# 101001000/ElevenRender

Hardware: AMD Instinct MI355X
Metric: Msamples/sec (rays traced x bounces) at 1920x1080, 1M-tri scene (higher is better)
Workload: dtype f32; 1 GPU; C2: 1000000-triangle random soup + 2048x1024 sky HDRI, 1920x1080, max_bounces 8, 1 step = 1 spp pass (config total 256 spp), seed 12345; schedule=stream

## Files before the change

elevenrender_amd/abi.py:

```python
import ctypes as C
import os

import numpy as np

_HERE = os.path.dirname(os.path.abspath(__file__))
LIB_PATH = os.environ.get("ELEVEN_HIP_LIB") or os.path.join(_HERE, "libeleven_hip.so")

ER_OK = 0
ER_ERR_INVALID_ARG, ER_ERR_NO_DEVICE, ER_ERR_HIP, ER_ERR_STATE, ER_ERR_OOM = -1, -2, -3, -4, -5
PASS_BEAUTY, PASS_DENOISE, PASS_NORMAL, PASS_TANGENT, PASS_BITANGENT, PASS_COUNT = 0, 1, 2, 3, 4, 5
PASS_NAMES = {"beauty": 0, "denoise": 1, "normal": 2, "tangent": 3, "bitangent": 4}
FLAG_POINT_LIGHTS, FLAG_COUNTERS, FLAG_MEGAKERNEL, FLAG_PROFILE, FLAG_FUSED, FLAG_WAVEFRONT, FLAG_GPU_BUILD, FLAG_MIS, FLAG_STREAM = 1, 2, 4, 8, 16, 32, 64, 128, 256
FLAG_HOST_BUILD = 512
FLAG_MESH_LIGHTS = 1024


class ErVec3(C.Structure):
    _fields_ = [("x", C.c_float), ("y", C.c_float), ("z", C.c_float)]


class ErCamera(C.Structure):
    _fields_ = [("focal_length", C.c_float), ("sensor_width", C.c_float), ("sensor_height", C.c_float),
                ("aperture", C.c_float), ("focus_distance", C.c_float), ("rotation", ErVec3),
                ("bokeh", C.c_int32), ("position", ErVec3)]


class ErMaterial(C.Structure):
    _fields_ = [("albedo_tex", C.c_int32), ("emission_tex", C.c_int32), ("roughness_tex", C.c_int32),
                ("metallic_tex", C.c_int32), ("normal_tex", C.c_int32), ("opacity_tex", C.c_int32),
                ("transmission_tex", C.c_int32), ("albedo_shader_id", C.c_int32),
                ("albedo", ErVec3), ("emission", ErVec3),
                ("opacity", C.c_float), ("roughness", C.c_float), ("metallic", C.c_float),
                ("clearcoat_gloss", C.c_float), ("clearcoat", C.c_float), ("anisotropic", C.c_float),
                ("eta", C.c_float), ("transmission", C.c_float), ("specular", C.c_float),
                ("specular_tint", C.c_float), ("sheen_tint", C.c_float), ("subsurface", C.c_float),
                ("sheen", C.c_float), ("ax", C.c_float), ("ay", C.c_float)]


class ErTexture(C.Structure):
    _fields_ = [("width", C.c_int32), ("height", C.c_int32), ("channels", C.c_int32), ("filter", C.c_int32),
                ("data", C.POINTER(C.c_float))]


class ErHdri(C.Structure):
    _fields_ = [("texture", ErTexture), ("cdf", C.POINTER(C.c_float)), ("radiance_sum", C.c_float)]


class ErPointLight(C.Structure):
    _fields_ = [("position", ErVec3), ("radiance", ErVec3)]


class ErSceneDesc(C.Structure):
    _fields_ = [("tri_count", C.c_uint32),
                ("vertices", C.POINTER(C.c_float)), ("normals", C.POINTER(C.c_float)),
                ("tangents", C.POINTER(C.c_float)), ("uvs", C.POINTER(C.c_float)),
                ("tangent_sign", C.POINTER(C.c_float)), ("material_id", C.POINTER(C.c_int32)),
                ("material_count", C.c_uint32), ("materials", C.POINTER(ErMaterial)),
                ("texture_count", C.c_uint32), ("textures", C.POINTER(ErTexture)),
                ("hdri", ErHdri), ("camera", ErCamera),
                ("point_light_count", C.c_uint32), ("point_lights", C.POINTER(ErPointLight)),
                ("x_res", C.c_uint32), ("y_res", C.c_uint32)]


class ErRenderParams(C.Structure):
    _fields_ = [("sample_target", C.c_uint32), ("block_size", C.c_uint32), ("max_bounces", C.c_uint32),
                ("device", C.c_int32), ("rank", C.c_uint32), ("world", C.c_uint32), ("flags", C.c_uint32)]


class ErDeviceInfo(C.Structure):
    _fields_ = [("name", C.c_char * 256), ("platform", C.c_char * 64), ("memory_bytes", C.c_uint64),
                ("compute_units", C.c_uint32), ("compatible", C.c_int32), ("arch", C.c_char * 64)]


class ErCounters(C.Structure):
    _fields_ = [(n, C.c_uint64) for n in ("paths", "bounce_samples", "rays", "node_visits", "tri_tests",
                                          "shaded_hits", "texel_fetches", "hdri_samples", "trace_wave_steps", "trace_busy_lanes",
                                          "trace_node_lanes", "trace_tri_lanes")]


class ErProfile(C.Structure):
    _fields_ = [("trace_ms", C.c_float), ("shade_ms", C.c_float), ("trace_launches", C.c_uint32), ("shade_launches", C.c_uint32), ("schedule", C.c_uint32),
                ("concurrency", C.c_uint32), ("empty_launches", C.c_uint32), ("empty_ms", C.c_float), ("rays_logged", C.c_uint64)]


class ErAccelInfo(C.Structure):
    _fields_ = [("node_count", C.c_uint32), ("node_bytes", C.c_uint32), ("leaf_count", C.c_uint32),
                ("max_depth", C.c_uint32), ("tri_record_bytes", C.c_uint32), ("build_ms", C.c_float),
                ("upload_ms", C.c_float), ("lift_bound", C.c_float), ("builder", C.c_uint32)]


class ErAdaptiveParams(C.Structure):
    _fields_ = [("threshold", C.c_float), ("min_samples", C.c_uint32), ("interval", C.c_uint32)]


class ErAdaptiveInfo(C.Structure):
    _fields_ = [("enabled", C.c_uint32), ("owned_tiles", C.c_uint32), ("active_tiles", C.c_uint32), ("tests_done", C.c_uint32),
                ("samples_rendered", C.c_uint32), ("next_test", C.c_uint32), ("pixel_samples", C.c_uint64), ("max_active_error", C.c_float)]


class ErLightInfo(C.Structure):
    _fields_ = [("emitters", C.c_uint32), ("total_weight", C.c_float)]


class ErStreamInfo(C.Structure):
    _fields_ = [("waves", C.c_uint32), ("tracers", C.c_uint32), ("large_regions", C.c_uint32), ("deal_pending", C.c_uint32), ("launches", C.c_uint32),
                ("pixels_per_cu", C.c_uint32), ("lanes_busy", C.c_double), ("launch_ms", C.c_double), ("cost_spread", C.c_double),
                ("spec_started", C.c_uint64), ("spec_right", C.c_uint64), ("spec_wrong", C.c_uint64),
                ("form", C.c_uint32), ("reserved", C.c_uint32)]


class ErStreamForm(C.Structure):
    _fields_ = [("waves", C.c_uint32), ("tracers", C.c_uint32), ("adapt", C.c_uint32), ("keep", C.c_uint32), ("spec", C.c_uint32), ("reserved", C.c_uint32)]


class ErAccelDump(C.Structure):
    _fields_ = [("tri_count", C.c_uint32), ("node_count", C.c_uint32), ("node8_count", C.c_uint32), ("node8_pieces", C.c_uint32),
                ("attr_pieces", C.c_uint32), ("max_depth", C.c_uint32), ("max_depth8", C.c_uint32), ("builder", C.c_uint32),
                ("lo", C.c_float * 3), ("hi", C.c_float * 3), ("lift_bound", C.c_float), ("max_lift", C.c_float)]


NODE_DTYPE = np.dtype([("lo0", "<f4", 3), ("hi0", "<f4", 3), ("lo1", "<f4", 3), ("hi1", "<f4", 3), ("c0", "<i4"), ("c1", "<i4"), ("pad", "<i4", 2)])
NODE8_DTYPE = np.dtype([("p", "<f4", 3), ("e", "u1", 3), ("imask", "u1"), ("child_base", "<u4"), ("tri_base", "<u4"), ("tri_present", "<u4"),
                        ("reserved", "<u4"), ("qlo", "u1", (3, 8)), ("qhi", "u1", (3, 8))])
ISECT_DTYPE = np.dtype([("v0", "<f4", 3), ("tri_id", "<i4"), ("v1", "<f4", 3), ("lift", "<f4"), ("v2", "<f4", 3), ("sign", "<f4")])
assert NODE_DTYPE.itemsize == 64 and NODE8_DTYPE.itemsize == 80 and ISECT_DTYPE.itemsize == 48


def attr_dtype(pieces):
    dt = np.dtype([("n", "<f4", (3, 3)), ("t", "<f4", (3, 3)), ("uv", "<f4", (3, 2)), ("material", "<i4"), ("pad", "<u4", 4 * pieces - 25)])
    assert dt.itemsize == 16 * pieces
    return dt


def accel_dump_dict(info, **arrays):
    d = {n: int(getattr(info, n)) for n in ("tri_count", "node_count", "node8_count", "max_depth", "max_depth8", "builder")}
    d["lo"], d["hi"] = np.array(list(info.lo), np.float32), np.array(list(info.hi), np.float32)
    d["lift_bound"], d["max_lift"] = np.float32(info.lift_bound), np.float32(info.max_lift)
    d.update(arrays)
    return d


def debug_bvh_dump(vertices, normals, threads=0):
    lib = load()
    v = np.ascontiguousarray(vertices, np.float32).reshape(-1, 3, 3)
    nn = np.ascontiguousarray(normals, np.float32).reshape(-1, 3, 3)
    assert v.shape == nn.shape
    n = len(v)
    info = ErAccelDump()
    args = (_fptr(v), _fptr(nn), n, threads, C.byref(info))
    check(lib.er_debug_bvh_dump(*args, None, 0, None, 0, None, 0, None, 0))
    assert info.node8_pieces * 16 == NODE8_DTYPE.itemsize
    nodes, nodes8 = np.zeros(info.node_count, NODE_DTYPE), np.zeros(info.node8_count, NODE8_DTYPE)
    s2t, lift = np.zeros(n, np.uint32), np.zeros(n, np.float32)
    vp = lambda a: a.ctypes.data_as(C.c_void_p)
    check(lib.er_debug_bvh_dump(*args, vp(nodes), nodes.nbytes, vp(nodes8), nodes8.nbytes, s2t.ctypes.data_as(C.POINTER(C.c_uint32)), s2t.nbytes,
                                _fptr(lift), lift.nbytes))
    return accel_dump_dict(info, nodes=nodes, nodes8=nodes8, slot_to_tri=s2t, tri_lift=lift)


class ErTraceRec(C.Structure):
    _fields_ = [("bounce", C.c_int32), ("tri", C.c_int32), ("shadow_tri", C.c_int32), ("opaque", C.c_int32),
                ("position", C.c_float * 3), ("wi", C.c_float * 3), ("light", C.c_float * 3), ("reduction", C.c_float * 3),
                ("shadow_occ", C.c_int32), ("light_occ", C.c_int32)]


_P = C.c_void_p
_FP, _IP = C.POINTER(C.c_float), C.POINTER(C.c_int32)
SYMBOLS = {
    "er_abi_version": (C.c_int, []),
    "er_last_error": (C.c_char_p, []),
    "er_device_count": (C.c_int, []),
    "er_device_info": (C.c_int, [C.c_int, C.POINTER(ErDeviceInfo)]),
    "er_device_find": (C.c_int, [C.c_char_p]),
    "er_scene_create": (C.c_int, [C.POINTER(ErSceneDesc), C.POINTER(_P)]),
    "er_scene_destroy": (None, [_P]),
    "er_render_begin": (C.c_int, [_P, C.POINTER(ErRenderParams)]),
    "er_render_samples": (C.c_int, [_P, C.c_uint32]),
    "er_render_samples_async": (C.c_int, [_P, C.c_uint32]),
    "er_wait": (C.c_int, [_P, C.POINTER(C.c_float)]),
    "er_samples_done": (C.c_int, [_P, C.POINTER(C.c_uint32)]),
    "er_read_pass": (C.c_int, [_P, C.c_int, C.POINTER(C.c_float)]),
    "er_read_samples": (C.c_int, [_P, C.POINTER(C.c_uint32)]),
    "er_read_rng": (C.c_int, [_P, C.POINTER(C.c_uint32)]),
    "er_owned_count": (C.c_int, [_P, C.c_uint32, C.POINTER(C.c_uint64)]),
    "er_pack_owned": (C.c_int, [_P, C.c_int, _P]),
    "er_unpack_owned": (C.c_int, [_P, C.c_int, C.c_uint32, _P]),
    "er_get_counters": (C.c_int, [_P, C.POINTER(ErCounters)]),
    "er_accel_info": (C.c_int, [_P, C.POINTER(ErAccelInfo)]),
    "er_adaptive_set": (C.c_int, [_P, C.POINTER(ErAdaptiveParams)]),
    "er_adaptive_info": (C.c_int, [_P, C.POINTER(ErAdaptiveInfo)]),
    "er_read_tile_state": (C.c_int, [_P, _FP, C.POINTER(C.c_uint32)]),
    "er_light_info": (C.c_int, [_P, C.POINTER(ErLightInfo)]),
    "er_get_profile": (C.c_int, [_P, C.POINTER(ErProfile)]),
    "er_denoise": (C.c_int, [_P, C.c_uint32, C.c_float]),
    "er_state_size": (C.c_int, [_P, C.POINTER(C.c_uint64)]),
    "er_state_export": (C.c_int, [_P, _P, C.c_uint64]),
    "er_state_import": (C.c_int, [_P, _P, C.c_uint64]),
    "er_comm_unique_id": (C.c_int, [C.POINTER(C.c_uint8)]),
    "er_comm_create": (C.c_int, [C.POINTER(C.c_uint8), C.c_uint32, C.c_uint32, C.c_int, C.POINTER(_P)]),
    "er_comm_destroy": (None, [_P]),
    "er_gather_pass": (C.c_int, [_P, C.c_int, _P, C.c_uint32]),
    "er_debug_comm_create_local": (C.c_int, [C.c_uint32, C.POINTER(_P)]),
    "er_comm_create_local": (C.c_int, [C.c_uint32, C.POINTER(_P)]),
    "er_debug_stream_info": (C.c_int, [_P, C.POINTER(ErStreamInfo)]),
    "er_debug_gather_buffers": (C.c_int, [_P, C.c_uint32, C.POINTER(_P), C.POINTER(C.c_uint64), C.POINTER(_P), C.POINTER(C.c_uint64)]),
    "er_debug_comm_loopback": (C.c_int, [_P, C.c_uint64, C.POINTER(C.c_double)]),
    "er_measure_hbm_peak": (C.c_int, [C.c_int, C.c_uint64, C.c_uint32, _FP, _FP]),
    "er_debug_eval": (C.c_int, [_P, C.c_int, _FP, C.c_uint32, C.c_uint32, _FP, C.c_uint32]),
    "er_debug_trace_rays": (C.c_int, [_P, _FP, _FP, C.c_uint32, _IP, _FP, _IP, _IP, _FP, _FP, _IP]),
    "er_debug_trace_pixel": (C.c_int, [_P, C.c_uint32, C.POINTER(ErTraceRec), C.c_int, C.POINTER(C.c_int)]),
    "er_debug_read_light_table": (C.c_int, [_P, _IP, _FP, C.c_uint32]),
    "er_debug_set_host_alloc_limit": (None, [C.c_uint64]),
    "er_debug_set_gpu_build_failure": (None, [C.c_int]),
    "er_debug_closest_hit": (C.c_int, [_P, C.POINTER(C.c_float), C.POINTER(C.c_float), C.c_uint32, C.POINTER(C.c_int32), C.POINTER(C.c_float),
                                       C.POINTER(C.c_float)]),
}

_lib = None


class ErError(RuntimeError):
    def __init__(self, code, msg):
        super().__init__(f"eleven_hip error {code}: {msg}")
        self.code = code


ABI_VERSION = 2

OPTIONAL_SYMBOLS = {
    "er_debug_stream_form": (C.c_int, [C.c_uint32, C.c_uint32, C.c_int, C.c_uint32, C.c_uint32, C.POINTER(ErStreamForm)]),
    "er_debug_read_accel": (C.c_int, [_P, C.POINTER(ErAccelDump), _P, C.c_uint64, _P, C.c_uint64, _P, C.c_uint64, _P, C.c_uint64]),
    "er_debug_bvh_dump": (C.c_int, [_FP, _FP, C.c_uint32, C.c_int, C.POINTER(ErAccelDump), _P, C.c_uint64, _P, C.c_uint64, C.POINTER(C.c_uint32), C.c_uint64,
                                    _FP, C.c_uint64]),
}


def load():
    global _lib
    if _lib is not None:
        return _lib
    if not os.path.exists(LIB_PATH):
        raise ErError(ER_ERR_NO_DEVICE, f"{LIB_PATH} is missing: the HIP extension is not built "
                      "(run __graft_entry__.build()); there is no CPU fallback")
    lib = C.CDLL(LIB_PATH)
    for name, (res, args) in SYMBOLS.items():
        fn = getattr(lib, name)
        fn.restype = res
        fn.argtypes = args
    for name, (res, args) in OPTIONAL_SYMBOLS.items():
        if hasattr(lib, name):
            getattr(lib, name).restype, getattr(lib, name).argtypes = res, args
    if lib.er_abi_version() != ABI_VERSION:
        raise ErError(ER_ERR_STATE, f"{LIB_PATH} has ABI version {lib.er_abi_version()}, this binding was written for {ABI_VERSION}: rebuild")
    _lib = lib
    return lib


def check(rc):
    if rc != ER_OK:
        raise ErError(rc, load().er_last_error().decode("utf-8", "replace"))


def _fptr(a):
    return a.ctypes.data_as(C.POINTER(C.c_float))


def _f32(a, shape=None):
    a = np.ascontiguousarray(a, dtype=np.float32)
    if shape is not None:
        a = a.reshape(shape)
    return a


class SceneData:

    def __init__(self, vertices, normals, tangents, uvs, tangent_sign, material_id, materials,
                 textures=(), hdri=None, hdri_cdf=None, hdri_radiance_sum=0.0, camera=None,
                 x_res=64, y_res=64, point_lights=()):
        n = 0 if vertices is None else int(np.asarray(vertices).size // 9)
        self.tri_count = n
        self.vertices = _f32(vertices if n else np.zeros((0, 3, 3)), (n, 3, 3))
        self.normals = _f32(normals if n else np.zeros((0, 3, 3)), (n, 3, 3))
        self.tangents = _f32(tangents if n else np.zeros((0, 3, 3)), (n, 3, 3))
        self.uvs = _f32(uvs if n else np.zeros((0, 3, 2)), (n, 3, 2))
        self.tangent_sign = _f32(tangent_sign if n else np.zeros((0,)), (n,))
        self.material_id = np.ascontiguousarray(material_id if n else np.zeros((0,)), dtype=np.int32).reshape(n)
        self.materials = list(materials)
        self.textures = [(_f32(d), int(w), int(h), int(ch), int(flt)) for (d, w, h, ch, flt) in textures]
        if hdri is None:
            hdri = (np.full((1, 1, 3), 0.5, np.float32), 1, 1, 3, 0)
        d, w, h, ch, flt = hdri
        self.hdri = (_f32(d), int(w), int(h), int(ch), int(flt))
        self.hdri_cdf = None if hdri_cdf is None else _f32(hdri_cdf)
        self.hdri_radiance_sum = float(hdri_radiance_sum)
        self.camera = camera if camera is not None else default_camera()
        self.x_res, self.y_res = int(x_res), int(y_res)
        self.point_lights = list(point_lights)
        self._desc = None

    def desc(self):
        if self._desc is not None:
            return self._desc
        d = ErSceneDesc()
        d.tri_count = self.tri_count
        d.vertices, d.normals, d.tangents = _fptr(self.vertices), _fptr(self.normals), _fptr(self.tangents)
        d.uvs, d.tangent_sign = _fptr(self.uvs), _fptr(self.tangent_sign)
        d.material_id = self.material_id.ctypes.data_as(C.POINTER(C.c_int32))
        self._mats = (ErMaterial * len(self.materials))(*self.materials)
        d.material_count, d.materials = len(self.materials), self._mats
        self._texs = (ErTexture * max(1, len(self.textures)))()
        for i, (data, w, h, ch, flt) in enumerate(self.textures):
            self._texs[i] = ErTexture(w, h, ch, flt, _fptr(data))
        d.texture_count, d.textures = len(self.textures), self._texs
        data, w, h, ch, flt = self.hdri
        d.hdri.texture = ErTexture(w, h, ch, flt, _fptr(data))
        if self.hdri_cdf is not None:
            d.hdri.cdf = _fptr(self.hdri_cdf)
            d.hdri.radiance_sum = self.hdri_radiance_sum
        d.camera = self.camera
        self._pls = (ErPointLight * max(1, len(self.point_lights)))(*self.point_lights)
        d.point_light_count, d.point_lights = len(self.point_lights), self._pls
        d.x_res, d.y_res = self.x_res, self.y_res
        self._desc = d
        return d


def default_camera():
    c = ErCamera()
    c.focal_length = 35 * 0.001
    c.sensor_width = 36 * 0.001
    c.sensor_height = 24 * 0.001
    c.aperture = 2.8
    c.focus_distance = 1000000.0
    c.rotation = ErVec3(0, 0, 0)
    c.bokeh = 0
    c.position = ErVec3(0, 0, 0)
    return c


def default_material(**kw):
    m = ErMaterial()
    for f in ("albedo_tex", "emission_tex", "roughness_tex", "metallic_tex", "normal_tex", "opacity_tex",
              "transmission_tex", "albedo_shader_id"):
        setattr(m, f, -1)
    m.albedo = ErVec3(0.5, 0.5, 0.5)
    m.emission = ErVec3(0, 0, 0)
    m.opacity, m.roughness, m.metallic = 1, 1, 0
    m.clearcoat_gloss = m.clearcoat = m.anisotropic = m.eta = m.transmission = 0
    m.specular, m.specular_tint, m.sheen_tint = 0.5, 0, 0.5
    m.subsurface = m.sheen = m.ax = m.ay = 0
    for k, v in kw.items():
        if isinstance(v, (tuple, list)):
            v = ErVec3(*v)
        setattr(m, k, v)
    return m
```

elevenrender_amd/csrc/er_api.cpp:

```cpp
#include <algorithm>
#include <chrono>

#include "er_scene.h"
#include <thread>
#include <system_error>

using namespace erh;

extern "C" {

int er_abi_version(void) { return ER_ABI_VERSION; }
const char* er_last_error(void) { return g_err.c_str(); }

int er_device_count(void) {
    int n = 0;
    if (hipGetDeviceCount(&n) != hipSuccess) return 0;
    return n;
}

static int er_device_info_impl(int index, ErDeviceInfo* out) {
    if (!out) return fail(ER_ERR_INVALID_ARG, "er_device_info: out is NULL");
    int n = er_device_count();
    if (index < 0 || index >= n) return fail(ER_ERR_NO_DEVICE, "er_device_info: no such HIP device");
    hipDeviceProp_t p;
// ... 210 lines not shown
        host_reserve((uint64_t)n * (sizeof(ErTriIsect) * 2 + sizeof(ErTriAttr) + 2 * sizeof(ErNode)));
        const ErBvhBuild& bvh = B.bvh;
        er_build_bvh(s->vertices.data(), s->normals.data(), s->tri_count, 0, &B.bvh);
        g.n8_pieces = bvh.nodes8.size() * ER_NODE8_PIECES + 8;
        g.nodes_f4 = bvh.nodes.size() * 4; g.geom_f4 = g.n8_pieces + (n + 1) * 3; g.attr_f4 = n * ER_ATTR_PIECES;
        g.nodes8_count = (uint32_t)bvh.nodes8.size(); g.max_depth8 = bvh.max_depth8; g.max_depth2 = bvh.max_depth; g.leaf_count = bvh.leaf_count;
        for (int a = 0; a < 3; a++) { g.lo[a] = bvh.lo[a]; g.hi[a] = bvh.hi[a]; }
        g.lift_bound = bvh.lift_bound;
        g.build_ms = bvh.build_ms;
    }
    HIP_TRY(hipEventRecord(built_ev, s->stream));
    if (g.max_depth2 > ER_BVH_MAX_DEPTH) return fail(ER_ERR_STATE, "er_render_begin: BVH deeper than the traversal stack");
    if (g.max_depth8 > ER_STACK8) return fail(ER_ERR_STATE, "er_render_begin: wide BVH deeper than the traversal stack (ER_STACK8)");
    if (g.geom_f4 >= (1ull << 30)) return fail(ER_ERR_INVALID_ARG, "er_render_begin: geometry exceeds the 16 GB addressable by the wide traversal");
    s->accel.builder = built ? 1u : 0u;
    return built ? ER_OK : accel_upload_host(s, B, g);
}

int begin_materials(ErScene* s, BeginStaging& B) {
    int rc;
    if ((rc = upload(s->d_materials, s->materials.data(), s->materials.size(), s->stream)) != ER_OK) return rc;
    std::vector<float4>& mat_pre = B.mat_pre;
    mat_pre.resize(s->materials.size());
    for (size_t i = 0; i < s->materials.size(); i++) {
        const ErMaterial& m = s->materials[i];
        const float a = 0.1f + m.clearcoat_gloss * (0.001f - 0.1f);
        const float a2 = a * a;
        mat_pre[i] = make_float4(ermath::er_pow(m.roughness, 2.2f), ermath::er_pow(m.metallic, 2.2f), a < 1.0f ? ermath::er_log(a2) : 0.0f, a < 1.0f ? 1.0f : 0.0f);
    }
    if (getenv("ER_MAT_PRE_ON_DEVICE")) for (auto& v : mat_pre) v.w = 0.0f;
    if ((rc = upload(s->d_mat_pre, mat_pre.data(), mat_pre.size(), s->stream)) != ER_OK) return rc;
    return upload(s->d_lights, s->point_lights.data(), s->point_lights.size(), s->stream);
}

int begin_textures(ErScene* s, BeginStaging& B, TexResult& out) {
    int rc;
    std::vector<DevTex>& table = B.table;
    std::vector<float>& pool = B.pool;
    std::vector<DevFused>& fused = B.fused;
    std::vector<uint8_t> vec_use(s->textures.size(), 0), scal_use(s->textures.size(), 0), plain_use(s->textures.size(), 0);
    auto mark = [&](std::vector<uint8_t>& v, int32_t id) { if (id >= 0 && (size_t)id < v.size()) v[(size_t)id] = 1; };
    for (const ErMaterial& m : s->materials) {
        mark(vec_use, m.albedo_tex); mark(vec_use, m.emission_tex); mark(vec_use, m.normal_tex);
        mark(scal_use, m.opacity_tex); mark(scal_use, m.roughness_tex); mark(scal_use, m.metallic_tex); mark(scal_use, m.transmission_tex);
        mark(plain_use, m.opacity_tex); mark(plain_use, m.transmission_tex);
    }
    const char* compact_knob = getenv("ER_TEX_COMPACT");
    const bool compact = !(compact_knob && atoi(compact_knob) == 0);
    table.resize(s->textures.size());
    const bool pow_on_host = !getenv("ER_MAT_PRE_ON_DEVICE");
    std::vector<uint8_t> mode(s->textures.size(), 0);
    for (size_t i = 0; i < s->textures.size(); i++) {
        const HostTex& t = s->textures[i];
        if (compact && t.channels >= 1 && scal_use[i] && !vec_use[i]) {
            const bool powered = t.filter != 1 && !plain_use[i] && pow_on_host;
            if (t.channels > 1 || powered) mode[i] = powered ? 2 : 1;
        }
    }
    s->tex_mode = mode;
    std::vector<std::vector<float>> one(s->textures.size());
    for (size_t i = 0; i < s->textures.size(); i++)
        if (mode[i]) one[i].resize((size_t)s->textures[i].width * (size_t)s->textures[i].height);
    {
        std::atomic<size_t> next{0};
        auto work = [&]() noexcept {
            for (size_t i = next.fetch_add(1); i < s->textures.size(); i = next.fetch_add(1)) {
                if (!mode[i]) continue;
                const HostTex& t = s->textures[i];
                const size_t n = one[i].size();
                for (size_t k = 0; k < n; k++) {
                    const float v = t.data[k * (size_t)t.channels];
                    one[i][k] = mode[i] == 2 ? ermath::er_pow(v, 2.2f) : v;
                }
            }
        };
        const unsigned nt = std::min<unsigned>(8u, std::max(1u, std::thread::hardware_concurrency()));
        struct JoinAll {
            std::vector<std::thread> th;
            ~JoinAll() { for (auto& x : th) if (x.joinable()) x.join(); }
        } pool_threads;
        pool_threads.th.reserve(nt);
        try {
            for (unsigned k = 1; k < nt; k++) pool_threads.th.emplace_back(work);
        } catch (const std::system_error&) {
        }
        work();
    }
    for (size_t i = 0; i < s->textures.size(); i++) {
        const HostTex& t = s->textures[i];
        if (mode[i]) {
            table[i] = DevTex{t.width, t.height, 1, mode[i] == 2 ? 2 : (t.filter == 1 ? 1 : 0), (uint32_t)pool.size()};
            pool.insert(pool.end(), one[i].begin(), one[i].end());
            std::vector<float>().swap(one[i]);
            continue;
        }
        table[i] = DevTex{t.width, t.height, t.channels, t.filter == 1 ? 1 : 0, (uint32_t)pool.size()};
        pool.insert(pool.end(), t.data.begin(), t.data.end());
    }
    fused.assign(std::max<size_t>(1, s->materials.size()), DevFused{0, 0, 0, 0});
    const char* fuse_knob = getenv("ER_TEX_FUSE");
    if (compact && !(fuse_knob && atoi(fuse_knob) == 0)) {
        for (size_t m = 0; m < s->materials.size(); m++) {
            const ErMaterial& M = s->materials[m];
            const int32_t ids[3] = {M.albedo_tex, M.roughness_tex, M.metallic_tex};
            bool ok = true;
            for (int32_t id : ids) ok = ok && id >= 0 && (size_t)id < s->textures.size();
            if (!ok) continue;
            const HostTex &A = s->textures[(size_t)ids[0]], &R = s->textures[(size_t)ids[1]], &K = s->textures[(size_t)ids[2]];
            if (A.width != R.width || A.width != K.width || A.height != R.height || A.height != K.height) continue;
            if ((A.filter == 1) != (R.filter == 1) || (A.filter == 1) != (K.filter == 1)) continue;
            if (A.channels < 1 || R.channels < 1 || K.channels < 1) continue;
            const bool bilinear = A.filter == 1, powered = !bilinear && pow_on_host;
            const size_t n = (size_t)A.width * (size_t)A.height;
            if (pool.size() + 5 * n >= (1ull << 32)) continue;
            fused[m] = DevFused{A.width, A.height, bilinear ? 1 : (powered ? 2 : 0), (uint32_t)pool.size()};
            const DevTex tr = table[(size_t)ids[1]], tk = table[(size_t)ids[2]];
            const bool r_done = powered && tr.filter == 2, k_done = powered && tk.filter == 2;
            for (size_t k = 0; k < n; k++) {
                const float* a = A.data.data() + k * (size_t)A.channels;
                const float r = r_done ? pool[tr.offset + k] : R.data[k * (size_t)R.channels], mt = k_done ? pool[tk.offset + k] : K.data[k * (size_t)K.channels];
                pool.push_back(a[0]);
                pool.push_back(A.channels == 1 ? a[0] : a[1]);
                pool.push_back(A.channels == 1 ? a[0] : (A.channels == 2 ? 0.0f : a[2]));
                pool.push_back(powered && !r_done ? ermath::er_pow(r, 2.2f) : r);
                pool.push_back(powered && !k_done ? ermath::er_pow(mt, 2.2f) : mt);
            }
        }
    }
    s->fused_any = false;
    for (const DevFused& f : fused) s->fused_any = s->fused_any || f.width > 0;
    if ((rc = upload(s->d_mat_fused, fused.data(), fused.size(), s->stream)) != ER_OK) return rc;
    out.hdri = DevTex{s->hdri_tex.width, s->hdri_tex.height, s->hdri_tex.channels, s->hdri_tex.filter, (uint32_t)pool.size()};
    pool.insert(pool.end(), s->hdri_tex.data.begin(), s->hdri_tex.data.end());
    if (pool.size() >= (1ull << 32)) return fail(ER_ERR_INVALID_ARG, "er_render_begin: texture pool exceeds 2^32 floats");
    if ((rc = upload(s->d_textures, table.data(), table.size(), s->stream)) != ER_OK) return rc;
    if ((rc = upload(s->d_tex_pool, pool.data(), pool.size(), s->stream)) != ER_OK) return rc;
    if ((rc = upload(s->d_cdf, s->hdri_cdf.data(), s->hdri_cdf.size(), s->stream)) != ER_OK) return rc;
    out.buckets = er_build_cdf_guide(s->hdri_cdf.data(), s->hdri_tex.width * s->hdri_tex.height, B.guide);
    return upload(s->d_guide, B.guide.data(), B.guide.size(), s->stream);
}

int begin_emitters(ErScene* s, BeginStaging& B, size_t n8_pieces, bool point_lights_on) {
    if (!(s->params.flags & ER_FLAG_MESH_LIGHTS)) return ER_OK;
    int rc;
    std::vector<int32_t>& etex = B.etex;
    for (const ErMaterial& m : s->materials)
        if (m.emission_tex >= 0 && (size_t)m.emission_tex < s->textures.size()) etex.push_back(m.emission_tex);
    std::sort(etex.begin(), etex.end());
    etex.erase(std::unique(etex.begin(), etex.end()), etex.end());
    ScopedDevBuf<int32_t> d_etex;
    if ((rc = upload(d_etex, etex.data(), etex.size(), s->stream)) != ER_OK) return rc;
    float* tab = nullptr;
    HIP_TRY(er_lights_build(s->d_nodes8.p + n8_pieces, s->d_attr.p, s->tri_count, s->d_materials.p, s->d_textures.p, s->d_tex_pool.p, d_etex.p,
                            (uint32_t)etex.size(), (uint32_t)s->textures.size(), &tab, &s->light_emitters, &s->light_total, s->stream));
    s->d_light_tab.p = tab;
    s->d_light_tab.n = tab ? (size_t)s->tri_count + 2 * (size_t)s->light_emitters : 0;
    if (point_lights_on && s->light_emitters > 0)
        return fail(ER_ERR_INVALID_ARG, "er_render_begin: ER_FLAG_POINT_LIGHTS and ER_FLAG_MESH_LIGHTS on a scene with both point lights and "
                                        "emissive triangles: both need the one light-query record per slot");
    return ER_OK;
}

int begin_planes(ErScene* s, BeginStaging& B) {
    int rc;
    const size_t npx = (size_t)s->x_res * s->y_res;
    if ((rc = upload(s->d_passes, nullptr, npx * ER_PASS_COUNT, s->stream)) != ER_OK) return rc;
    if ((rc = upload(s->d_samples, nullptr, npx, s->stream)) != ER_OK) return rc;
    if ((rc = upload(s->d_rng, nullptr, npx, s->stream)) != ER_OK) return rc;
    B.owned = s->tiles_of(s->params.rank, s->params.world);
    if ((rc = upload(s->d_owned, B.owned.data(), B.owned.size(), s->stream)) != ER_OK) return rc;
    if ((rc = upload(s->d_counters, nullptr, 1, s->stream)) != ER_OK) return rc;
    HIP_TRY(hipMemsetAsync(s->d_counters.p, 0, sizeof(DevCounters), s->stream));
    return ER_OK;
}

int begin_choose_schedule(ErScene* s, BeginStaging& B, uint32_t cus) {
    const uint32_t all = ER_FLAG_MEGAKERNEL | ER_FLAG_FUSED | ER_FLAG_WAVEFRONT | ER_FLAG_STREAM;
    uint32_t forced = s->params.flags & all;
    if (forced == ER_FLAG_FUSED) forced = ER_FLAG_STREAM;
    if (forced & (forced - 1)) return fail(ER_ERR_INVALID_ARG, "er_render_begin: more than one schedule flag");
    uint32_t sched = forced;
    if (forced == 0 || forced == ER_FLAG_STREAM) B.deal = stream_deal_owned(B.owned, s->tiles_x(), cus);
    if (forced == 0) {
        sched = ((size_t)B.deal.most * 64u > ER_STREAM_MAX_RING || s->x_res > 65535u || s->y_res > 65535u) ? ER_FLAG_WAVEFRONT : ER_FLAG_STREAM;
    }
    s->params.flags = (s->params.flags & ~all) | sched;
    return ER_OK;
}

int begin_wavefront(ErScene* s, const std::vector<uint32_t>& owned, uint32_t cus, bool query_on) {
    int rc;
    uint32_t pools = 3;
    if (const char* e = getenv("ER_WF_POOLS")) pools = (uint32_t)std::min(8, std::max(1, atoi(e)));
    pools = std::min<uint32_t>(pools, std::max<uint32_t>(1u, (uint32_t)owned.size()));
    const size_t pool_tiles = (owned.size() + pools - 1) / pools;
    const size_t qcap = pool_tiles * 64;
    size_t slots = owned.size() * 64;
    const size_t sh = query_on ? 2 : 1;
    const size_t qs_cap = qcap * sh;
    const size_t q_words = 2 * qcap + 2 * qs_cap;
    if ((rc = upload(s->d_wf4, nullptr, slots * (7 + 4 * sh), s->stream)) != ER_OK) return rc;
    if ((rc = upload(s->d_wf1, nullptr, slots * (3 + 3 * sh) + q_words * pools + (size_t)WF_COUNTS * pools, s->stream)) != ER_OK) return rc;
    WfState W{};
    float4* f = s->d_wf4.p;
    W.ray_o = f; W.ray_d = f + slots; W.light = f + 2 * slots; W.reduc = f + 3 * slots;
    W.aov_n = f + 4 * slots; W.aov_t = f + 5 * slots; W.aov_b = f + 6 * slots;
    W.sh_o = f + 7 * slots; W.sh_d = W.sh_o + sh * slots; W.c_vis = W.sh_d + sh * slots; W.c_occ = W.c_vis + sh * slots;
    uint32_t* u = s->d_wf1.p;
    W.hit = (int*)u; W.left = u + slots; W.hit2 = (int*)(u + 2 * slots);
    W.occluded = (int*)(u + 3 * slots); W.occ_a = W.occluded + sh * slots; W.occ_b = W.occ_a + sh * slots;
    uint32_t* qbase = u + (3 + 3 * sh) * slots;
    uint32_t* cbase = qbase + q_words * pools;
    W.pools = pools;
    W.slots = (uint32_t)slots;
    s->trace_blocks = cus * 12;
    s->shade_blocks = cus * 5;
    if (const char* e = getenv("ER_TRACE_WAVES_PER_CU")) s->trace_blocks = cus * (uint32_t)std::max(1, atoi(e));
    if (const char* e = getenv("ER_SHADE_WAVES_PER_CU")) s->shade_blocks = cus * (uint32_t)std::max(1, atoi(e));
    const size_t trace_spill = (size_t)s->trace_blocks * ER_STACK8 * 64;
    const size_t spill_per_pool = trace_spill + (size_t)s->shade_blocks * ER_BVH_MAX_DEPTH * 32;
    if ((rc = upload(s->d_spill, nullptr, spill_per_pool * pools, s->stream)) != ER_OK) return rc;
    s->wf.clear();
    for (uint32_t p2 = 0; p2 < pools; p2++) {
        W.pool = p2;
        uint32_t* q = qbase + (size_t)p2 * q_words;
        W.q[0] = q; W.q[1] = q + qcap; W.qs[0] = q + 2 * qcap; W.qs[1] = q + 2 * qcap + qs_cap;
        W.counts = cbase + (size_t)p2 * WF_COUNTS;
        W.spill = s->d_spill.p + (size_t)p2 * spill_per_pool;
        W.shade_stack = (int*)(W.spill + trace_spill);
        s->wf.push_back(W);
    }
    for (uint32_t p2 = 1; p2 < pools; p2++) {
        hipStream_t st;
        HIP_TRY(hipStreamCreateWithFlags(&st, hipStreamNonBlocking));
        s->pool_streams.push_back(st);
    }
    for (uint32_t p2 = 0; p2 < pools; p2++) {
        hipEvent_t e;
        HIP_TRY(hipEventCreateWithFlags(&e, hipEventDisableTiming));
        s->pool_events.push_back(e);
    }
    return ER_OK;
}

int begin_descriptor(ErScene* s, const ErGpuBvhDevice& g, const TexResult& tex, uint32_t owned_tiles) {
    const float lift_bound = g.lift_bound;
    float scene_scale = 0;
    for (int a = 0; a < 3; a++) scene_scale = std::max(scene_scale, std::max(std::fabs(g.lo[a]), std::fabs(g.hi[a])));
    scene_scale = std::max(scene_scale, std::max(std::fabs(s->camera.position.x), std::max(std::fabs(s->camera.position.y), std::fabs(s->camera.position.z))));

    DevScene& D = s->dev;
    memset(&D, 0, sizeof(D));
    D.nodes = s->d_nodes.p;
    D.nodes8 = s->d_nodes8.p;
    D.tri_isect = s->d_nodes8.p + g.n8_pieces;
    D.tri_base_pieces = (uint32_t)g.n8_pieces;
    D.tri_attr = s->d_attr.p;
    D.tri_count = s->tri_count;
    D.node_count = (uint32_t)(g.nodes_f4 / 4);
    D.node8_count = g.nodes8_count;
    D.prune_margin = lift_bound + 1e-5f * scene_scale;
    D.max_lift = lift_bound;
    D.scene_scale = scene_scale;
    D.materials = s->d_materials.p;
    D.mat_pre = s->d_mat_pre.p;
    D.textures = s->d_textures.p;
    D.tex_pool = s->d_tex_pool.p;
    D.mat_fused = s->d_mat_fused.p;
    D.fused_any = s->fused_any ? 1u : 0u;
    D.hdri_tex = tex.hdri;
    D.hdri_cdf = s->d_cdf.p;
    D.hdri_guide = s->d_guide.p;
    D.hdri_buckets = tex.buckets;
    D.hdri_radiance_sum = s->hdri_radiance_sum;
    D.cam = s->camera;
    D.x_res = s->x_res;
    D.y_res = s->y_res;
    D.tiles_x = s->tiles_x();
    D.tiles_y = s->tiles_y();
    D.max_bounces = s->params.max_bounces;
    {
        auto pow2 = [](int32_t v) { return v > 0 && (v & (v - 1)) == 0; };
        bool all = pow2(tex.hdri.width) && pow2(tex.hdri.height);
        for (const HostTex& t : s->textures) all = all && pow2(t.width) && pow2(t.height);
        D.tex_pow2 = all ? 1u : 0u;
        if (const char* e = getenv("ER_TEX_POW2")) D.tex_pow2 = (atoi(e) != 0 && all) ? 1u : 0u;
    }
    D.trace_every_query = 0u;
    if (const char* e = getenv("ER_TRACE_EVERY_QUERY")) D.trace_every_query = atoi(e) != 0 ? 1u : 0u;
    D.ext_flags = s->params.flags & (ER_FLAG_POINT_LIGHTS | ER_FLAG_MIS);
    D.lights = s->d_lights.p;
    D.light_count = (uint32_t)s->point_lights.size();
    if (s->light_emitters > 0) {
        D.ext_flags = (D.ext_flags & ~(uint32_t)ER_FLAG_POINT_LIGHTS) | ER_FLAG_MESH_LIGHTS;
        D.mesh_lights = s->d_light_tab.p;
        D.emitter_count = s->light_emitters;
    }
    D.passes = s->d_passes.p;
    D.samples = s->d_samples.p;
    D.rng = s->d_rng.p;
    D.owned_tiles = s->d_owned.p;
    D.owned_tile_count = owned_tiles;
    D.counters = s->d_counters.p;
    D.tile_cost = ((s->params.flags & ER_FLAG_STREAM) && s->st.deal_pending) ? s->st.d_tile_cost.p : nullptr;
    D.px_draws = (s->params.flags & ER_FLAG_STREAM) ? s->st.d_px_draws.p : nullptr;
    {
        const erd::CamTrig t = erd::camera_trig(D.cam);
        D.cam_cx = t.cx; D.cam_sx = t.sx; D.cam_cy = t.cy; D.cam_sy = t.sy; D.cam_cz = t.cz; D.cam_sz = t.sz;
        D.cam_trig_valid = getenv("ER_CAM_TRIG_ON_DEVICE") ? 0u : 1u;
    }
    return upload(s->d_dev, &D, 1, s->stream);
}

}

static int er_render_begin_impl(ErScene* s, const ErRenderParams* p) {
    if (!s || !p) return fail(ER_ERR_INVALID_ARG, "er_render_begin: NULL argument");
    std::lock_guard<std::mutex> lk(s->mtx);
    int rc;
    ErDeviceInfo info;
    if ((rc = begin_check(p, info)) != ER_OK) return rc;
    if ((rc = begin_open(s, p)) != ER_OK) return rc;
    const uint32_t cus = std::max(1u, info.compute_units);
    EventPair ev;
    HIP_TRY(hipEventCreate(&ev.a));
    HIP_TRY(hipEventCreate(&ev.b));
    BeginStaging B;
    ErGpuBvhDevice g;
    TexResult tex;
    if ((rc = begin_accel(s, B, ev.a, g)) != ER_OK) return rc;
    if ((rc = begin_materials(s, B)) != ER_OK) return rc;
    const bool lights_on = (p->flags & ER_FLAG_POINT_LIGHTS) != 0 && !s->point_lights.empty();
    if ((rc = begin_textures(s, B, tex)) != ER_OK) return rc;
    if ((rc = begin_emitters(s, B, g.n8_pieces, lights_on)) != ER_OK) return rc;
    const bool query_on = lights_on || s->light_emitters > 0;
    if ((rc = begin_planes(s, B)) != ER_OK) return rc;
    if ((rc = begin_choose_schedule(s, B, cus)) != ER_OK) return rc;
    if (s->params.flags & ER_FLAG_STREAM) rc = stream_begin(s, B.owned, B.deal, cus, query_on);
    else if (s->params.flags & ER_FLAG_WAVEFRONT) rc = begin_wavefront(s, B.owned, cus, query_on);
    if (rc != ER_OK) return rc;
    HIP_TRY(hipEventRecord(ev.b, s->stream));
    if ((rc = begin_descriptor(s, g, tex, (uint32_t)B.owned.size())) != ER_OK) return rc;

    er_launch_setup(s->dev, s->stream);
    HIP_TRY(hipGetLastError());
    HIP_TRY(hipStreamSynchronize(s->stream));
    float up_ms = 0;
    (void)hipEventElapsedTime(&up_ms, ev.a, ev.b);

    s->accel.node_count = g.nodes8_count;
    s->accel.node_bytes = sizeof(ErNode8);
    s->accel.max_depth = g.max_depth8;
    s->accel.leaf_count = g.leaf_count;
    s->accel.tri_record_bytes = sizeof(ErTriIsect);
    s->accel.build_ms = (float)g.build_ms;
    s->accel.upload_ms = up_ms;
    s->accel.lift_bound = g.lift_bound;
    for (int a = 0; a < 3; a++) { s->accel_lo[a] = g.lo[a]; s->accel_hi[a] = g.hi[a]; }
    s->accel_depth2 = g.max_depth2;
    s->begun = true;
    return ER_OK;
}

static int wavefront_enqueue(ErScene* s, const DevScene& D, uint32_t n, bool count) {
    const uint32_t iters = n * (s->params.max_bounces + 1);
    const uint32_t pools = (uint32_t)s->wf.size();
    const bool prof = (s->params.flags & ER_FLAG_PROFILE) != 0;
    if (prof) {
        const size_t need = s->prof_used / 3 + (size_t)iters * pools;
        while (s->prof_events.size() < 3 * need) {
            hipEvent_t e;
            HIP_TRY(hipEventCreate(&e));
            s->prof_events.push_back(e);
        }
        if (s->d_ray_log.n < need) {
            DevBuf<uint32_t> bigger;
            int rc2 = upload(bigger, nullptr, need * 2, s->stream);
            if (rc2 != ER_OK) return rc2;
            if (s->d_ray_log.p && s->prof_used) {
                HIP_TRY(hipStreamSynchronize(s->stream));
                HIP_TRY(hipMemcpy(bigger.p, s->d_ray_log.p, (s->prof_used / 3) * sizeof(uint32_t), hipMemcpyDeviceToDevice));
            }
            s->d_ray_log.release();
            s->d_ray_log = bigger;
        }
    }
    if (pools > 1) {
        HIP_TRY(hipEventRecord(s->pool_events[0], s->stream));
        for (uint32_t p = 1; p < pools; p++) HIP_TRY(hipStreamWaitEvent(s->pool_streams[p - 1], s->pool_events[0], 0));
    }
    auto pool_stream = [&](uint32_t p) { return p == 0 ? s->stream : s->pool_streams[p - 1]; };
    for (uint32_t p = 0; p < pools; p++) er_launch_wf_begin(D, s->wf[p], n, pool_stream(p));
    for (uint32_t it = 0; it < iters; it++) {
        for (uint32_t p = 0; p < pools; p++) {
            hipStream_t st = pool_stream(p);
            uint32_t* ray_log = prof ? s->d_ray_log.p + s->prof_used / 3 : nullptr;
            if (prof) HIP_TRY(hipEventRecord(s->prof_events[s->prof_used++], st));
            er_launch_wf_trace(D, s->wf[p], it & 1, count, s->trace_blocks, ray_log, st);
            if (prof) HIP_TRY(hipEventRecord(s->prof_events[s->prof_used++], st));
            er_launch_wf_shade(D, s->wf[p], it & 1, count, s->shade_blocks, st);
            if (prof) HIP_TRY(hipEventRecord(s->prof_events[s->prof_used++], st));
        }
    }
    for (uint32_t p = 1; p < pools; p++) {
        HIP_TRY(hipEventRecord(s->pool_events[p], s->pool_streams[p - 1]));
        HIP_TRY(hipStreamWaitEvent(s->stream, s->pool_events[p], 0));
    }
    return ER_OK;
}

static int enqueue_samples(ErScene* s, uint32_t n) {
    const DevScene& D = s->ad_on ? s->ad_dev : s->dev;
    const bool count = (s->params.flags & ER_FLAG_COUNTERS) != 0;
    int rc = ER_OK;
    if (!(s->params.flags & (ER_FLAG_MEGAKERNEL | ER_FLAG_STREAM))) {
        if (n > 0) rc = wavefront_enqueue(s, D, n, count);
    } else {
        const bool prof = (s->params.flags & ER_FLAG_PROFILE) && n > 0;
        if (prof) {
            while (s->prof_events.size() < s->prof_used + 3) {
                hipEvent_t e;
                HIP_TRY(hipEventCreate(&e));
                s->prof_events.push_back(e);
            }
            HIP_TRY(hipEventRecord(s->prof_events[s->prof_used++], s->stream));
        }
        if (s->params.flags & ER_FLAG_STREAM) rc = stream_enqueue(s, n);
        else er_launch_render(D, n, count, s->stream);
        if (rc == ER_OK && prof) {
            HIP_TRY(hipEventRecord(s->prof_events[s->prof_used++], s->stream));
            HIP_TRY(hipEventRecord(s->prof_events[s->prof_used++], s->stream));
        }
    }
    if (rc != ER_OK) return rc;
    HIP_TRY(hipGetLastError());
    return ER_OK;
}

static int adaptive_render(ErScene* s, uint32_t n);

static int er_render_samples_async_impl(ErScene* s, uint32_t n) {
    if (!s) return fail(ER_ERR_INVALID_ARG, "er_render_samples: NULL scene");
    std::lock_guard<std::mutex> lk(s->mtx);
    if (!s->begun) return fail(ER_ERR_STATE, "er_render_samples: er_render_begin has not succeeded");
    if ((s->params.flags & ER_FLAG_STREAM) && n >= (1u << 24))
        return fail(ER_ERR_INVALID_ARG, "er_render_samples: at most 16777215 samples per call in the streaming schedule");
    HIP_TRY(hipSetDevice(s->device));
    if (!s->timing_open) {
        HIP_TRY(hipEventRecord(s->ev_start, s->stream));
        s->timing_open = true;
    }
    if (n > 0) for (auto& u : s->unpacked) u.clear();
    if (s->ad_on) return adaptive_render(s, n);
    s->rendered += n;
    return enqueue_samples(s, n);
}

static int er_wait_impl(ErScene* s, float* elapsed_ms) {
    if (!s) return fail(ER_ERR_INVALID_ARG, "er_wait: NULL scene");
    std::lock_guard<std::mutex> lk(s->mtx);
    if (!s->begun) return fail(ER_ERR_STATE, "er_wait: er_render_begin has not succeeded");
    HIP_TRY(hipSetDevice(s->device));
    float ms = 0;
    if (s->timing_open) {
        HIP_TRY(hipEventRecord(s->ev_stop, s->stream));
        HIP_TRY(hipEventSynchronize(s->ev_stop));
        HIP_TRY(hipEventElapsedTime(&ms, s->ev_start, s->ev_stop));
        s->timing_open = false;
    } else {
        HIP_TRY(hipStreamSynchronize(s->stream));
    }
    if (elapsed_ms) *elapsed_ms = ms;
    { int rc = er_scene_stream_status(s, "er_wait"); if (rc != ER_OK) { s->prof_used = 0; return rc; } }
    stream_adapt(s);
    s->profile = ErProfile{};
    s->profile.schedule = s->params.flags & (ER_FLAG_MEGAKERNEL | ER_FLAG_WAVEFRONT | ER_FLAG_STREAM);
    s->profile.concurrency = (s->params.flags & ER_FLAG_WAVEFRONT) ? (uint32_t)std::max<size_t>(1, s->wf.size()) : 1u;
    std::vector<uint32_t> ray_log;
    const bool wf = (s->params.flags & ER_FLAG_WAVEFRONT) != 0;
    if (wf && s->prof_used && s->d_ray_log.p) {
        ray_log.resize(s->prof_used / 3);
        HIP_TRY(hipMemcpy(ray_log.data(), s->d_ray_log.p, ray_log.size() * sizeof(uint32_t), hipMemcpyDeviceToHost));
    }
    for (size_t i = 0; i + 2 < s->prof_used; i += 3) {
        float a = 0, b = 0;
        HIP_TRY(hipEventElapsedTime(&a, s->prof_events[i], s->prof_events[i + 1]));
        HIP_TRY(hipEventElapsedTime(&b, s->prof_events[i + 1], s->prof_events[i + 2]));
        if (wf && i / 3 < ray_log.size() && ray_log[i / 3] == 0) {
            s->profile.empty_launches++;
            s->profile.empty_ms += a + b;
            continue;
        }
        s->profile.trace_ms += a;
        s->profile.shade_ms += b;
        s->profile.trace_launches++;
        s->profile.shade_launches++;
        if (wf && i / 3 < ray_log.size()) s->profile.rays_logged += ray_log[i / 3];
    }
    s->prof_used = 0;
    return ER_OK;
}

static int er_render_samples_impl(ErScene* s, uint32_t n) {
    int rc = er_render_samples_async(s, n);
    if (rc != ER_OK) return rc;
    return er_wait(s, nullptr);
}

static int read_back_locked(ErScene* s, const void* src, void* dst, size_t bytes, const char* who) {
    if (!s->begun) return fail(ER_ERR_STATE, std::string(who) + ": er_render_begin has not succeeded");
    HIP_TRY(hipSetDevice(s->device));
    HIP_TRY(hipMemcpyAsync(dst, src, bytes, hipMemcpyDeviceToHost, s->stream));
    HIP_TRY(hipStreamSynchronize(s->stream));
    return er_scene_stream_status(s, who);
}

static int read_back(ErScene* s, const void* src, void* dst, size_t bytes, const char* who) {
    if (!s || !dst) return fail(ER_ERR_INVALID_ARG, std::string(who) + ": NULL argument");
    std::lock_guard<std::mutex> lk(s->mtx);
    return read_back_locked(s, src, dst, bytes, who);
}

static int er_samples_done_impl(ErScene* s, uint32_t* out) {
    if (!s) return fail(ER_ERR_INVALID_ARG, "er_samples_done: NULL scene");
    uint32_t first = 0;
    std::unique_lock<std::mutex> lk(s->mtx);
    if (s->begun && s->params.world > 1) {
        std::vector<uint32_t> t = s->tiles_of(s->params.rank, s->params.world);
        if (!t.empty()) {
            const uint32_t tiles_x = s->tiles_x();
            first = (t[0] / tiles_x) * ER_TILE * s->x_res + (t[0] % tiles_x) * ER_TILE;
        }
    }
    lk.unlock();
    return read_back(s, s->d_samples.p + first, out, sizeof(uint32_t), "er_samples_done");
}

static int er_read_pass_impl(ErScene* s, int pass, float* dst) {
    if (pass < 0 || pass >= ER_PASS_COUNT) return fail(ER_ERR_INVALID_ARG, "er_read_pass: pass out of range");
    if (!s) return fail(ER_ERR_INVALID_ARG, "er_read_pass: NULL scene");
    if (!dst) return fail(ER_ERR_INVALID_ARG, "er_read_pass: NULL argument");
    std::lock_guard<std::mutex> lk(s->mtx);
    if (!s->begun) return fail(ER_ERR_STATE, "er_read_pass: er_render_begin has not succeeded");
    size_t npx = (size_t)s->x_res * s->y_res;
    HIP_TRY(hipSetDevice(s->device));
    int rc;
    if (s->d_plane.n < npx && (rc = upload(s->d_plane, nullptr, npx, s->stream)) != ER_OK) return rc;
    er_launch_plane(s->dev, pass, s->d_plane.p, s->stream);
    HIP_TRY(hipGetLastError());
    return read_back_locked(s, s->d_plane.p, dst, npx * sizeof(float4), "er_read_pass");
}
namespace {
struct StateHeader {
    char magic[8];
    uint32_t x_res, y_res, passes, reserved;
    uint64_t bytes;
    uint8_t pad[32];
};
static_assert(sizeof(StateHeader) == 64, "snapshot header is 64 bytes");
uint64_t state_bytes(const ErScene* s) {
    const uint64_t npx = (uint64_t)s->x_res * s->y_res;
    return sizeof(StateHeader) + npx * (ER_PASS_COUNT * sizeof(float4) + 2 * sizeof(uint32_t));
}
}

static int er_state_size_impl(ErScene* s, uint64_t* bytes) {
    if (!s || !bytes) return fail(ER_ERR_INVALID_ARG, "er_state_size: NULL argument");
    *bytes = state_bytes(s);
    return ER_OK;
}

static int er_state_export_impl(ErScene* s, void* dst, uint64_t bytes) {
    if (!s || !dst) return fail(ER_ERR_INVALID_ARG, "er_state_export: NULL argument");
    std::lock_guard<std::mutex> lk(s->mtx);
    if (!s->begun) return fail(ER_ERR_STATE, "er_state_export: er_render_begin has not succeeded");
    if (bytes < state_bytes(s)) return fail(ER_ERR_INVALID_ARG, "er_state_export: buffer smaller than er_state_size");
    HIP_TRY(hipSetDevice(s->device));
    const size_t npx = (size_t)s->x_res * s->y_res;
    StateHeader h{};
    memcpy(h.magic, "ERSTATE2", 8);
    h.x_res = s->x_res; h.y_res = s->y_res; h.passes = ER_PASS_COUNT; h.bytes = state_bytes(s);
    uint8_t* p = (uint8_t*)dst;
    memcpy(p, &h, sizeof(h));
    p += sizeof(h);
    HIP_TRY(hipMemcpyAsync(p, s->d_passes.p, npx * ER_PASS_COUNT * sizeof(float4), hipMemcpyDeviceToHost, s->stream));
    p += npx * ER_PASS_COUNT * sizeof(float4);
    HIP_TRY(hipMemcpyAsync(p, s->d_samples.p, npx * sizeof(uint32_t), hipMemcpyDeviceToHost, s->stream));
    p += npx * sizeof(uint32_t);
    HIP_TRY(hipMemcpyAsync(p, s->d_rng.p, npx * sizeof(uint32_t), hipMemcpyDeviceToHost, s->stream));
    HIP_TRY(hipStreamSynchronize(s->stream));
    return er_scene_stream_status(s, "er_state_export");
}

static int er_state_import_impl(ErScene* s, const void* src, uint64_t bytes) {
    if (!s || !src) return fail(ER_ERR_INVALID_ARG, "er_state_import: NULL argument");
    std::lock_guard<std::mutex> lk(s->mtx);
    if (!s->begun) return fail(ER_ERR_STATE, "er_state_import: er_render_begin has not succeeded");
    if (s->ad_on) return fail(ER_ERR_STATE, "er_state_import: resuming an adaptive render is not supported (er_adaptive_set)");
    StateHeader h;
    if (bytes < sizeof(h)) return fail(ER_ERR_INVALID_ARG, "er_state_import: truncated snapshot");
    memcpy(&h, src, sizeof(h));
    if (memcmp(h.magic, "ERSTATE2", 8) != 0) return fail(ER_ERR_INVALID_ARG, "er_state_import: not a snapshot of this library version (bad magic)");
    if (h.x_res != s->x_res || h.y_res != s->y_res || h.passes != ER_PASS_COUNT)
        return fail(ER_ERR_INVALID_ARG, "er_state_import: the snapshot is of a " + std::to_string(h.x_res) + "x" + std::to_string(h.y_res) + " frame");
    if (h.bytes != state_bytes(s) || bytes < h.bytes) return fail(ER_ERR_INVALID_ARG, "er_state_import: truncated snapshot");
    HIP_TRY(hipSetDevice(s->device));
    const size_t npx = (size_t)s->x_res * s->y_res;
// ... 305 lines not shown
```

elevenrender_amd/csrc/er_debug_api.cpp:

```cpp
#include "er_scene.h"
#include "er_debug.h"

using namespace erh;

#include "../../include/eleven_hip_debug.h"

static int er_debug_closest_hit_impl(ErScene* s, const float* origins, const float* dirs, uint32_t n, int32_t* tri_ids, float* positions, float* distances) {
    if (!s || !origins || !dirs || !tri_ids || !positions || !distances) return fail(ER_ERR_INVALID_ARG, "er_debug_closest_hit: NULL argument");
    std::lock_guard<std::mutex> lk(s->mtx);
    if (!s->begun) return fail(ER_ERR_STATE, "er_debug_closest_hit: er_render_begin has not succeeded");
    HIP_TRY(hipSetDevice(s->device));
    ScopedDevBuf<float> d_o, d_d, d_pos, d_dist;
    ScopedDevBuf<int32_t> d_tri;
    int rc;
    if ((rc = upload(d_o, origins, (size_t)n * 3, s->stream)) != ER_OK) return rc;
    if ((rc = upload(d_d, dirs, (size_t)n * 3, s->stream)) != ER_OK) return rc;
    if ((rc = upload(d_pos, (const float*)nullptr, (size_t)n * 3, s->stream)) != ER_OK) return rc;
    if ((rc = upload(d_dist, (const float*)nullptr, (size_t)n, s->stream)) != ER_OK) return rc;
    if ((rc = upload(d_tri, (const int32_t*)nullptr, (size_t)n, s->stream)) != ER_OK) return rc;
    er_launch_debug_hit(s->dev, d_o.p, d_d.p, n, d_tri.p, d_pos.p, d_dist.p, s->stream);
    HIP_TRY(hipGetLastError());
    HIP_TRY(hipMemcpyAsync(tri_ids, d_tri.p, (size_t)n * 4, hipMemcpyDeviceToHost, s->stream));
    HIP_TRY(hipMemcpyAsync(positions, d_pos.p, (size_t)n * 12, hipMemcpyDeviceToHost, s->stream));
    HIP_TRY(hipMemcpyAsync(distances, d_dist.p, (size_t)n * 4, hipMemcpyDeviceToHost, s->stream));
    HIP_TRY(hipStreamSynchronize(s->stream));
    return ER_OK;
}

static int er_debug_cdf_search_impl(const float* cdf, int length, const float* values, int32_t* out, int count) {
    if (!cdf || !values || !out || length <= 0) return fail(ER_ERR_INVALID_ARG, "er_debug_cdf_search: bad argument");
    std::vector<uint32_t> guide;
    int buckets = er_build_cdf_guide(cdf, length, guide);
    for (int i = 0; i < count; i++) out[i] = er_cdf_search(cdf, length, guide.data(), buckets, values[i]);
    return ER_OK;
}

static int er_debug_stream_deal_impl(const uint32_t* owned, uint32_t count, uint32_t tiles_x, uint32_t blocks, int xcd_aware, uint32_t edge, uint32_t* out, uint32_t out_cap,
                                     uint32_t* most) {
    if ((count && !owned) || !tiles_x || !blocks || !most) return fail(ER_ERR_INVALID_ARG, "er_debug_stream_deal: bad argument");
    std::vector<uint32_t> deal;
    *most = er_stream_deal_tiles(owned, count, tiles_x, blocks, xcd_aware != 0, deal, edge);
    if (deal.size() > out_cap || (deal.size() && !out)) return fail(ER_ERR_INVALID_ARG, "er_debug_stream_deal: out holds fewer than blocks * most entries");
    for (size_t i = 0; i < deal.size(); i++) out[i] = deal[i];
    return ER_OK;
}

static int er_debug_stream_form_impl(uint32_t tiles, uint32_t blocks, int light_query, uint32_t tri_count, uint32_t flags, ErStreamForm* out) {
    if (!out || !blocks) return fail(ER_ERR_INVALID_ARG, "er_debug_stream_form: bad argument");
    const StreamForm f = stream_choose_form(tiles, blocks, light_query != 0, tri_count, flags);
    *out = ErStreamForm{f.waves, f.tracers, f.adapt ? 1u : 0u, f.keep ? 1u : 0u, f.spec ? 1u : 0u, 0u};
    return ER_OK;
}

static int er_debug_bvh_check_impl(const float* vertices, const float* normals, uint32_t tri_count, int threads, ErBvhCheck* out) {
    if (!out || (tri_count && (!vertices || !normals))) return fail(ER_ERR_INVALID_ARG, "er_debug_bvh_check: NULL argument");
    ErBvhBuild b;
    er_build_bvh(vertices, normals, tri_count, threads, &b);
    memset(out, 0, sizeof(*out));
    out->node_count = (uint32_t)b.nodes.size();
    out->leaf_count = b.leaf_count;
    out->max_depth = b.max_depth;
    out->lift_bound = b.lift_bound;
    out->build_ms = (float)b.build_ms;
    std::vector<uint8_t> seen(tri_count, 0), visited(b.nodes.size(), 0);
    struct Item { int32_t ref; float lo[3], hi[3]; bool has_box; };
    std::vector<Item> stack;
    if (!b.nodes.empty()) stack.push_back(Item{0, {0, 0, 0}, {0, 0, 0}, false});
    auto area = [](const float* lo, const float* hi) {
        float x = hi[0] - lo[0], y = hi[1] - lo[1], z = hi[2] - lo[2];
        return 2.0 * ((double)x * y + (double)x * z + (double)y * z);
    };
    double root_area = 0;
    if (!b.nodes.empty()) {
        const ErNode& r = b.nodes[0];
        float lo[3], hi[3];
        for (int a = 0; a < 3; a++) {
            lo[a] = r.c1 == ER_BVH_NO_CHILD ? r.lo0[a] : std::min(r.lo0[a], r.lo1[a]);
            hi[a] = r.c1 == ER_BVH_NO_CHILD ? r.hi0[a] : std::max(r.hi0[a], r.hi1[a]);
        }
        root_area = area(lo, hi);
    }
    while (!stack.empty()) {
        Item it = stack.back();
        stack.pop_back();
        if (it.ref == ER_BVH_NO_CHILD) continue;
        if (it.ref >= 0) {
            if ((size_t)it.ref >= b.nodes.size()) { out->uncontained++; continue; }
            if (visited[it.ref]++) { out->duplicate_tris++; continue; }
            const ErNode& n = b.nodes[it.ref];
            const float* los[2] = {n.lo0, n.lo1};
            const float* his[2] = {n.hi0, n.hi1};
            const int32_t cs[2] = {n.c0, n.c1};
            for (int k = 0; k < 2; k++) {
                if (cs[k] == ER_BVH_NO_CHILD) continue;
                if (it.has_box)
                    for (int a = 0; a < 3; a++)
                        if (los[k][a] < it.lo[a] || his[k][a] > it.hi[a]) out->uncontained++;
                Item c;
                c.ref = cs[k];
                c.has_box = true;
                memcpy(c.lo, los[k], 12);
                memcpy(c.hi, his[k], 12);
                uint32_t cnt = 0;
                if (cs[k] < 0) cnt = ((uint32_t)~cs[k] & 7u) + 1;
                if (root_area > 0) out->sah_cost += area(los[k], his[k]) / root_area * (cs[k] < 0 ? cnt : 1.0);
                stack.push_back(c);
            }
        } else {
            uint32_t v = (uint32_t)~it.ref, first = v >> 3, cnt = (v & 7u) + 1;
            out->max_leaf_size = std::max(out->max_leaf_size, cnt);
            for (uint32_t i = 0; i < cnt; i++) {
                uint32_t slot = first + i;
                if (slot >= tri_count) { out->uncontained++; continue; }
                uint32_t id = b.slot_to_tri[slot];
                if (seen[id]++) out->duplicate_tris++;
                out->tris_in_leaves++;
                for (int k = 0; k < 3; k++)
                    for (int a = 0; a < 3; a++) {
                        float p = vertices[(size_t)id * 9 + k * 3 + a];
                        if (p < it.lo[a] || p > it.hi[a]) out->uncontained++;
                    }
            }
        }
    }
    for (uint8_t v : visited) if (!v) out->unreachable_nodes++;
    return ER_OK;
}

static int dump_put(const char* who, void* dst, uint64_t cap, const void* src, uint64_t bytes, bool from_device, hipStream_t st) {
    if (!dst) return ER_OK;
    if (cap < bytes) return fail(ER_ERR_INVALID_ARG, std::string(who) + ": a buffer is smaller than its array (all buffers NULL queries the sizes)");
    if (!bytes) return ER_OK;
    if (from_device) HIP_TRY(hipMemcpyAsync(dst, src, bytes, hipMemcpyDeviceToHost, st));
    else memcpy(dst, src, bytes);
    return ER_OK;
}

static int er_debug_read_accel_impl(ErScene* s, ErAccelDump* info, void* nodes, uint64_t nodes_cap, void* nodes8, uint64_t nodes8_cap, void* isect, uint64_t isect_cap,
                                    void* attr, uint64_t attr_cap) {
    if (!s || !info) return fail(ER_ERR_INVALID_ARG, "er_debug_read_accel: NULL argument");
    std::lock_guard<std::mutex> lk(s->mtx);
    if (!s->begun) return fail(ER_ERR_STATE, "er_debug_read_accel: er_render_begin has not succeeded");
    const DevScene& D = s->dev;
    memset(info, 0, sizeof(*info));
    info->tri_count = s->tri_count;
    info->node_count = D.node_count;
    info->node8_count = D.node8_count;
    info->node8_pieces = ER_NODE8_PIECES;
    info->attr_pieces = ER_ATTR_PIECES;
    info->max_depth = s->accel_depth2;
    info->max_depth8 = s->accel.max_depth;
    info->builder = s->accel.builder;
    for (int a = 0; a < 3; a++) { info->lo[a] = s->accel_lo[a]; info->hi[a] = s->accel_hi[a]; }
    info->lift_bound = s->accel.lift_bound;
    info->max_lift = D.max_lift;
    if (!nodes && !nodes8 && !isect && !attr) return ER_OK;
    HIP_TRY(hipSetDevice(s->device));
    int rc;
    const char* who = "er_debug_read_accel";
    if ((rc = dump_put(who, nodes, nodes_cap, D.nodes, (uint64_t)D.node_count * sizeof(ErNode), true, s->stream)) != ER_OK) return rc;
    if ((rc = dump_put(who, nodes8, nodes8_cap, D.nodes8, (uint64_t)D.node8_count * ER_NODE8_PIECES * 16, true, s->stream)) != ER_OK) return rc;
    if ((rc = dump_put(who, isect, isect_cap, D.tri_isect, ((uint64_t)s->tri_count + 1) * sizeof(ErTriIsect), true, s->stream)) != ER_OK) return rc;
    if ((rc = dump_put(who, attr, attr_cap, D.tri_attr, (uint64_t)s->tri_count * sizeof(ErTriAttr), true, s->stream)) != ER_OK) return rc;
    HIP_TRY(hipStreamSynchronize(s->stream));
    return ER_OK;
}

static int er_debug_bvh_dump_impl(const float* vertices, const float* normals, uint32_t tri_count, int threads, ErAccelDump* info, void* nodes, uint64_t nodes_cap,
                                  void* nodes8, uint64_t nodes8_cap, uint32_t* slot_to_tri, uint64_t slot_cap, float* tri_lift, uint64_t lift_cap) {
    if (!info || (tri_count && (!vertices || !normals))) return fail(ER_ERR_INVALID_ARG, "er_debug_bvh_dump: NULL argument");
    ErBvhBuild b;
    er_build_bvh(vertices, normals, tri_count, threads, &b);
    memset(info, 0, sizeof(*info));
    info->tri_count = tri_count;
    info->node_count = (uint32_t)b.nodes.size();
    info->node8_count = (uint32_t)b.nodes8.size();
    info->node8_pieces = sizeof(ErNode8) / 16;
    info->max_depth = b.max_depth;
    info->max_depth8 = b.max_depth8;
    for (int a = 0; a < 3; a++) { info->lo[a] = b.lo[a]; info->hi[a] = b.hi[a]; }
    info->lift_bound = info->max_lift = b.lift_bound;
    if (!nodes && !nodes8 && !slot_to_tri && !tri_lift) return ER_OK;
    int rc;
    const char* who = "er_debug_bvh_dump";
    if ((rc = dump_put(who, nodes, nodes_cap, b.nodes.data(), (uint64_t)b.nodes.size() * sizeof(ErNode), false, nullptr)) != ER_OK) return rc;
    if ((rc = dump_put(who, nodes8, nodes8_cap, b.nodes8.data(), (uint64_t)b.nodes8.size() * sizeof(ErNode8), false, nullptr)) != ER_OK) return rc;
    if ((rc = dump_put(who, slot_to_tri, slot_cap, b.slot_to_tri.data(), (uint64_t)tri_count * 4, false, nullptr)) != ER_OK) return rc;
    return dump_put(who, tri_lift, lift_cap, b.tri_lift.data(), (uint64_t)tri_count * 4, false, nullptr);
}

static int er_debug_trace_rays_impl(ErScene* s, const float* origins, const float* dirs, uint32_t n, const int32_t* self_slots, const float* limits,
                                    int32_t* tri_ids, int32_t* slots, float* positions, float* distances, int32_t* info) {
    if (!s || !origins || !dirs || !tri_ids || !slots || !positions || !distances || !info || (self_slots && !limits))
        return fail(ER_ERR_INVALID_ARG, "er_debug_trace_rays: NULL argument");
    std::lock_guard<std::mutex> lk(s->mtx);
    if (!s->begun) return fail(ER_ERR_STATE, "er_debug_trace_rays: er_render_begin has not succeeded");
    HIP_TRY(hipSetDevice(s->device));
    ScopedDevBuf<float> d_o, d_d, d_pos, d_dist, d_lim;
    ScopedDevBuf<int32_t> d_tri, d_slot, d_info, d_self;
    ScopedDevBuf<uint2> d_spill;
    int rc;
    if ((rc = upload(d_o, origins, (size_t)n * 3, s->stream)) != ER_OK) return rc;
    if ((rc = upload(d_d, dirs, (size_t)n * 3, s->stream)) != ER_OK) return rc;
    if (self_slots) {
        for (uint32_t i = 0; i < n; i++)
            if (self_slots[i] < -1 || self_slots[i] >= (int32_t)s->tri_count) return fail(ER_ERR_INVALID_ARG, "er_debug_trace_rays: self slot out of range");
        if ((rc = upload(d_self, self_slots, (size_t)n, s->stream)) != ER_OK) return rc;
        if ((rc = upload(d_lim, limits, (size_t)n, s->stream)) != ER_OK) return rc;
    }
    if ((rc = upload(d_pos, (const float*)nullptr, (size_t)n * 3, s->stream)) != ER_OK) return rc;
    if ((rc = upload(d_dist, (const float*)nullptr, (size_t)n, s->stream)) != ER_OK) return rc;
    if ((rc = upload(d_tri, (const int32_t*)nullptr, (size_t)n, s->stream)) != ER_OK) return rc;
    if ((rc = upload(d_slot, (const int32_t*)nullptr, (size_t)n, s->stream)) != ER_OK) return rc;
    if ((rc = upload(d_info, (const int32_t*)nullptr, (size_t)n, s->stream)) != ER_OK) return rc;
    if ((rc = upload(d_spill, (const uint2*)nullptr, (size_t)((n + 63) / 64) * ER_STACK8 * 64, s->stream)) != ER_OK) return rc;
    er_launch_debug_trace(s->dev, d_o.p, d_d.p, n, self_slots ? d_self.p : nullptr, self_slots ? d_lim.p : nullptr, d_tri.p, d_slot.p, d_pos.p,
                          d_dist.p, d_info.p, d_spill.p, s->stream);
    HIP_TRY(hipGetLastError());
    HIP_TRY(hipMemcpyAsync(tri_ids, d_tri.p, (size_t)n * 4, hipMemcpyDeviceToHost, s->stream));
    HIP_TRY(hipMemcpyAsync(slots, d_slot.p, (size_t)n * 4, hipMemcpyDeviceToHost, s->stream));
    HIP_TRY(hipMemcpyAsync(info, d_info.p, (size_t)n * 4, hipMemcpyDeviceToHost, s->stream));
    HIP_TRY(hipMemcpyAsync(positions, d_pos.p, (size_t)n * 12, hipMemcpyDeviceToHost, s->stream));
    HIP_TRY(hipMemcpyAsync(distances, d_dist.p, (size_t)n * 4, hipMemcpyDeviceToHost, s->stream));
    HIP_TRY(hipStreamSynchronize(s->stream));
    return ER_OK;
}

static int er_debug_trace_pixel_impl(ErScene* s, uint32_t idx, ErTraceRec* recs, int max_recs, int* count) {
    if (!s || !recs || !count || max_recs <= 0) return fail(ER_ERR_INVALID_ARG, "er_debug_trace_pixel: bad argument");
    std::lock_guard<std::mutex> lk(s->mtx);
    if (!s->begun) return fail(ER_ERR_STATE, "er_debug_trace_pixel: er_render_begin has not succeeded");
    if (idx >= s->x_res * s->y_res) return fail(ER_ERR_INVALID_ARG, "er_debug_trace_pixel: pixel index out of range");
    HIP_TRY(hipSetDevice(s->device));
    ScopedDevBuf<ErTraceRec> d_recs;
    ScopedDevBuf<int> d_count;
    ScopedDevBuf<uint2> d_spill;
    int rc;
    if ((rc = upload(d_recs, (const ErTraceRec*)nullptr, (size_t)max_recs, s->stream)) != ER_OK) return rc;
    if ((rc = upload(d_count, (const int*)nullptr, 1, s->stream)) != ER_OK) return rc;
    if ((rc = upload(d_spill, (const uint2*)nullptr, (size_t)ER_DEBUG_PIXEL_SCRATCH, s->stream)) != ER_OK) return rc;
    er_launch_debug_pixel(s->dev, idx, d_recs.p, max_recs, d_count.p, d_spill.p, s->stream);
    HIP_TRY(hipGetLastError());
    HIP_TRY(hipMemcpyAsync(count, d_count.p, sizeof(int), hipMemcpyDeviceToHost, s->stream));
    HIP_TRY(hipStreamSynchronize(s->stream));
    if (*count > 0) HIP_TRY(hipMemcpy(recs, d_recs.p, sizeof(ErTraceRec) * (size_t)*count, hipMemcpyDeviceToHost));
    return ER_OK;
}

static int er_debug_read_light_table_impl(ErScene* s, int32_t* tri_index, float* cdf, uint32_t cap) {
    if (!s) return fail(ER_ERR_INVALID_ARG, "er_debug_read_light_table: NULL scene");
    std::lock_guard<std::mutex> lk(s->mtx);
    if (!s->begun) return fail(ER_ERR_STATE, "er_debug_read_light_table: er_render_begin has not succeeded");
    const uint32_t m = std::min(cap, s->light_emitters);
    if (m == 0) return ER_OK;
    HIP_TRY(hipSetDevice(s->device));
    ScopedDevBuf<int32_t> d_tri;
    ScopedDevBuf<float> d_cdf;
    int rc;
    if ((rc = upload(d_tri, (const int32_t*)nullptr, m, s->stream)) != ER_OK) return rc;
    if ((rc = upload(d_cdf, (const float*)nullptr, m, s->stream)) != ER_OK) return rc;
    er_launch_light_table_read(s->dev.tri_isect, s->d_light_tab.p, s->tri_count, s->light_emitters, m, d_tri.p, d_cdf.p, s->stream);
    HIP_TRY(hipGetLastError());
    if (tri_index) HIP_TRY(hipMemcpyAsync(tri_index, d_tri.p, sizeof(int32_t) * m, hipMemcpyDeviceToHost, s->stream));
    if (cdf) HIP_TRY(hipMemcpyAsync(cdf, d_cdf.p, sizeof(float) * m, hipMemcpyDeviceToHost, s->stream));
    HIP_TRY(hipStreamSynchronize(s->stream));
    return ER_OK;
}

static int er_debug_eval_impl(ErScene* s, int kind, const float* in, uint32_t n, uint32_t in_stride, float* out, uint32_t out_stride) {
    static const uint32_t need_in[ER_FN_COUNT] = {1, 7, 7, 29, 29, 29, 3, 2, 4, 1, 2, 3};
    static const uint32_t need_out[ER_FN_COUNT] = {32, 6, 18, 3, 1, 3, 2, 3, 3, 1, 1, 1};
    if (!s || !in || !out) return fail(ER_ERR_INVALID_ARG, "er_debug_eval: NULL argument");
    if (kind < 0 || kind >= ER_FN_COUNT) return fail(ER_ERR_INVALID_ARG, "er_debug_eval: unknown kind");
    if (in_stride < need_in[kind] || out_stride < need_out[kind]) return fail(ER_ERR_INVALID_ARG, "er_debug_eval: stride smaller than the kind's item");
    std::lock_guard<std::mutex> lk(s->mtx);
    if (!s->begun) return fail(ER_ERR_STATE, "er_debug_eval: er_render_begin has not succeeded");
    if (kind == ER_FN_TEXTURE)
        for (uint32_t i = 0; i < n; i++) {
            int32_t id;
            memcpy(&id, &in[(size_t)i * in_stride], 4);
            if (id < -1 || id >= (int32_t)s->textures.size()) return fail(ER_ERR_INVALID_ARG, "er_debug_eval: texture id out of range");
            if (id >= 0 && (size_t)id < s->tex_mode.size() && s->tex_mode[(size_t)id] != 0)
                return fail(ER_ERR_STATE, "er_debug_eval: texture " + std::to_string(id) + " is kept compacted on the device (first channel" +
                                              (s->tex_mode[(size_t)id] == 2 ? ", to the power 2.2" : "") + "); begin the render with ER_TEX_COMPACT=0 to evaluate ER_FN_TEXTURE on it");
        }
    HIP_TRY(hipSetDevice(s->device));
    ScopedDevBuf<float> d_in, d_out;
    int rc;
    if ((rc = upload(d_in, in, (size_t)n * in_stride, s->stream)) != ER_OK) return rc;
    if ((rc = upload(d_out, (const float*)nullptr, (size_t)n * out_stride, s->stream)) != ER_OK) return rc;
    HIP_TRY(hipMemsetAsync(d_out.p, 0, std::max<size_t>((size_t)n * out_stride, 1) * sizeof(float), s->stream));
    er_launch_debug_eval(s->dev, kind, d_in.p, n, in_stride, d_out.p, out_stride, s->stream);
    HIP_TRY(hipGetLastError());
    HIP_TRY(hipMemcpyAsync(out, d_out.p, (size_t)n * out_stride * sizeof(float), hipMemcpyDeviceToHost, s->stream));
    HIP_TRY(hipStreamSynchronize(s->stream));
    return ER_OK;
}

static int er_measure_hbm_peak_impl(int device, uint64_t bytes, uint32_t iters, float* copy_GBps, float* read_GBps) {
    if (!copy_GBps || !read_GBps) return fail(ER_ERR_INVALID_ARG, "er_measure_hbm_peak: NULL argument");
    int ndev = er_device_count();
    if (device < 0 || device >= ndev) return fail(ER_ERR_NO_DEVICE, "er_measure_hbm_peak: no such HIP device");
    if (bytes == 0) bytes = 2ull << 30;
    if (iters == 0) iters = 5;
    HIP_TRY(hipSetDevice(device));
    const size_t n = (size_t)(bytes / 16);
    ScopedDevBuf<float4> a, b;
    ScopedDevBuf<float> sink;
    hipStream_t st = nullptr;
    HIP_TRY(hipStreamCreateWithFlags(&st, hipStreamNonBlocking));
    struct StreamGuard { hipStream_t s; ~StreamGuard() { (void)hipStreamDestroy(s); } } sg{st};
    int rc;
    if ((rc = upload(a, (const float4*)nullptr, n, st)) != ER_OK) return rc;
    if ((rc = upload(b, (const float4*)nullptr, n, st)) != ER_OK) return rc;
    if ((rc = upload(sink, (const float*)nullptr, 1, st)) != ER_OK) return rc;
    HIP_TRY(hipMemsetAsync(a.p, 0, n * 16, st));
    HIP_TRY(hipMemsetAsync(b.p, 0, n * 16, st));
    EventPair ev;
    HIP_TRY(hipEventCreate(&ev.a));
    HIP_TRY(hipEventCreate(&ev.b));
    float best_copy = 0, best_read = 0;
    for (uint32_t it = 0; it < iters + 1; it++) {
        float ms = 0;
        HIP_TRY(hipEventRecord(ev.a, st));
        er_launch_hbm_copy(a.p, b.p, n, st);
        HIP_TRY(hipEventRecord(ev.b, st));
        HIP_TRY(hipEventSynchronize(ev.b));
        HIP_TRY(hipEventElapsedTime(&ms, ev.a, ev.b));
        if (it > 0 && ms > 0) best_copy = std::max(best_copy, (float)(2.0 * n * 16 / (ms * 1e-3) / 1e9));
        HIP_TRY(hipEventRecord(ev.a, st));
        er_launch_hbm_read(a.p, sink.p, n, st);
        HIP_TRY(hipEventRecord(ev.b, st));
        HIP_TRY(hipEventSynchronize(ev.b));
        HIP_TRY(hipEventElapsedTime(&ms, ev.a, ev.b));
        if (it > 0 && ms > 0) best_read = std::max(best_read, (float)(1.0 * n * 16 / (ms * 1e-3) / 1e9));
    }
    HIP_TRY(hipGetLastError());
    *copy_GBps = best_copy;
    *read_GBps = best_read;
    return ER_OK;
}

extern "C" void er_debug_set_host_alloc_limit(uint64_t bytes) { g_host_alloc_limit.store(bytes); }


static int er_debug_stream_info_impl(ErScene* s, ErStreamInfo* out) {
    if (!s || !out) return fail(ER_ERR_INVALID_ARG, "er_debug_stream_info: NULL argument");
    std::lock_guard<std::mutex> lk(s->mtx);
    memset(out, 0, sizeof(*out));
    out->cost_spread = -1.0;
    if (!s->begun || !(s->params.flags & ER_FLAG_STREAM)) return ER_OK;
    stream_fill_info(s, out);
    return ER_OK;
}

extern "C" {
void er_debug_set_gpu_build_failure(int kind) { er_debug_gpu_build_failure.store(kind < 0 || kind > 3 ? 0 : kind); }
int er_debug_stream_info(ErScene* s, ErStreamInfo* out) { return guarded("er_debug_stream_info", [&]() -> int { return er_debug_stream_info_impl(s, out); }); }
int er_debug_closest_hit(ErScene* s, const float* origins, const float* dirs, uint32_t n, int32_t* tri_ids, float* positions, float* distances) { return guarded("er_debug_closest_hit", [&]() -> int { return er_debug_closest_hit_impl(s, origins, dirs, n, tri_ids, positions, distances); }); }
int er_debug_cdf_search(const float* cdf, int length, const float* values, int32_t* out, int count) { return guarded("er_debug_cdf_search", [&]() -> int { return er_debug_cdf_search_impl(cdf, length, values, out, count); }); }
int er_debug_stream_deal(const uint32_t* owned, uint32_t count, uint32_t tiles_x, uint32_t blocks, int xcd_aware, uint32_t edge, uint32_t* out, uint32_t out_cap, uint32_t* most) {
    return guarded("er_debug_stream_deal", [&]() -> int { return er_debug_stream_deal_impl(owned, count, tiles_x, blocks, xcd_aware, edge, out, out_cap, most); });
}
int er_debug_stream_form(uint32_t tiles, uint32_t blocks, int light_query, uint32_t tri_count, uint32_t flags, ErStreamForm* out) {
    return guarded("er_debug_stream_form", [&]() -> int { return er_debug_stream_form_impl(tiles, blocks, light_query, tri_count, flags, out); });
}
int er_debug_read_accel(ErScene* s, ErAccelDump* info, void* nodes, uint64_t nodes_cap, void* nodes8, uint64_t nodes8_cap, void* isect, uint64_t isect_cap, void* attr, uint64_t attr_cap) {
    return guarded("er_debug_read_accel", [&]() -> int { return er_debug_read_accel_impl(s, info, nodes, nodes_cap, nodes8, nodes8_cap, isect, isect_cap, attr, attr_cap); });
}
int er_debug_bvh_dump(const float* vertices, const float* normals, uint32_t tri_count, int threads, ErAccelDump* info, void* nodes, uint64_t nodes_cap, void* nodes8, uint64_t nodes8_cap,
                      uint32_t* slot_to_tri, uint64_t slot_cap, float* tri_lift, uint64_t lift_cap) {
    return guarded("er_debug_bvh_dump", [&]() -> int { return er_debug_bvh_dump_impl(vertices, normals, tri_count, threads, info, nodes, nodes_cap, nodes8, nodes8_cap, slot_to_tri, slot_cap, tri_lift, lift_cap); });
}
int er_debug_bvh_check(const float* vertices, const float* normals, uint32_t tri_count, int threads, ErBvhCheck* out) { return guarded("er_debug_bvh_check", [&]() -> int { return er_debug_bvh_check_impl(vertices, normals, tri_count, threads, out); }); }
int er_debug_trace_rays(ErScene* s, const float* origins, const float* dirs, uint32_t n, const int32_t* self_slots, const float* limits, int32_t* tri_ids,
                        int32_t* slots, float* positions, float* distances, int32_t* info) {
    return guarded("er_debug_trace_rays", [&]() -> int { return er_debug_trace_rays_impl(s, origins, dirs, n, self_slots, limits, tri_ids, slots, positions, distances, info); });
}
int er_debug_trace_pixel(ErScene* s, uint32_t idx, ErTraceRec* recs, int max_recs, int* count) {
    return guarded("er_debug_trace_pixel", [&]() -> int { return er_debug_trace_pixel_impl(s, idx, recs, max_recs, count); });
}
int er_debug_read_light_table(ErScene* s, int32_t* tri_index, float* cdf, uint32_t cap) {
    return guarded("er_debug_read_light_table", [&]() -> int { return er_debug_read_light_table_impl(s, tri_index, cdf, cap); });
}
int er_debug_eval(ErScene* s, int kind, const float* in, uint32_t n, uint32_t in_stride, float* out, uint32_t out_stride) {
    return guarded("er_debug_eval", [&]() -> int { return er_debug_eval_impl(s, kind, in, n, in_stride, out, out_stride); });
}
int er_measure_hbm_peak(int device, uint64_t bytes, uint32_t iters, float* copy_GBps, float* read_GBps) {
    return guarded("er_measure_hbm_peak", [&]() -> int { return er_measure_hbm_peak_impl(device, bytes, iters, copy_GBps, read_GBps); });
}
}
```

elevenrender_amd/csrc/er_stream.h:

```cpp
#pragma once
#include <hip/hip_runtime_api.h>
#include <stddef.h>
#include <stdint.h>

#include <vector>

struct DevScene;

#ifndef ER_STREAM_SLOTS
#define ER_STREAM_SLOTS 1024u
#endif

#ifndef ER_STREAM_SUPER_TILE_DEFAULT
#define ER_STREAM_SUPER_TILE_DEFAULT 8u
#endif
#ifndef ER_STREAM_SUPER_TILE_LARGE
#define ER_STREAM_SUPER_TILE_LARGE 16u
#endif
#ifndef ER_STREAM_COST_SPREAD_MAX
#define ER_STREAM_COST_SPREAD_MAX 0.04
#endif
#ifndef ER_STREAM_ADAPT_MIN_MS
#define ER_STREAM_ADAPT_MIN_MS 4.0
#endif
#ifndef ER_STREAM_SMALL_SHARE
#define ER_STREAM_SMALL_SHARE 1152u
#endif
#ifndef ER_STREAM_TEN_TRACERS_SHARE
#define ER_STREAM_TEN_TRACERS_SHARE 704u
#endif
#ifndef ER_STREAM_SPEC_SHARE
#define ER_STREAM_SPEC_SHARE 2304u
#endif
#ifndef ER_STREAM_SPEC_MIN_TRIS
#define ER_STREAM_SPEC_MIN_TRIS 1000u
#endif
#ifndef ER_STREAM_SPEC_LONG_DEFAULT
#define ER_STREAM_SPEC_LONG_DEFAULT 12
#endif
#ifndef ER_STREAM_KEEP_SHARE
#define ER_STREAM_KEEP_SHARE 6000u
#endif
#ifndef ER_STREAM_SPEC_KEEP_DEFAULT
#define ER_STREAM_SPEC_KEEP_DEFAULT 2
#endif
#define ER_STREAM_MAX_RING 32768u

enum ErStreamCtl : uint32_t {
    ER_SC_STATUS = 0,
    ER_SC_ITERS = 1,
    ER_SC_BUSY = 3,
    ER_SC_START = 5,
    ER_SC_END = 7,
    ER_SC_SPEC = 23,
    ER_SC_WORDS = 26
};
constexpr uint32_t ER_STREAM_CTL_LEAD = 1;
static_assert((ER_STREAM_CTL_LEAD + ER_SC_ITERS) % 2u == 0u && ER_SC_BUSY % 2u == 1u && ER_SC_START % 2u == 1u && ER_SC_END % 2u == 1u, "the 64-bit control words are 8-byte aligned");

struct ErStreamLaunch {
    const DevScene* S = nullptr;
    const DevScene* S_dev = nullptr;
    void* records = nullptr;
    uint32_t slots = 0;
    bool lights = false;
    void* spill = nullptr;
    const uint32_t* deal = nullptr;
    uint32_t deal_count = 0;
    void* ring = nullptr;
    uint32_t ring_cap = 0;
    uint32_t* status = nullptr;
    uint32_t n_samples = 0;
    bool count = false;
    uint32_t blocks = 0;
    uint32_t tracers = 0;
    uint32_t waves = 16;
    bool spec = false;
    bool keep = false;
    hipStream_t stream = nullptr;
};
void er_launch_stream_mesh(const ErStreamLaunch& L);
void er_launch_stream(const ErStreamLaunch& L);
struct ErStreamLaunchForm { uint32_t form, waves, bits; };
ErStreamLaunchForm er_stream_launch_form(uint32_t max_bounces, uint32_t tri_count, uint32_t waves, bool spec, bool keep);
uint32_t er_stream_deal_tiles(const uint32_t* owned, uint32_t count, uint32_t tiles_x, uint32_t blocks, bool xcd_aware, std::vector<uint32_t>& out, uint32_t edge = 0);
uint32_t er_stream_record_bytes(bool lights);
size_t er_stream_spill_entries(uint32_t blocks);
hipError_t er_probe_stream(const char** which);
```

elevenrender_amd/csrc/er_stream.hip:

```cpp
#include <algorithm>
#include <cstdlib>
#include "er_device.h"
#include "er_kernels.h"
#include "er_wavefront.h"
#include "er_trav.h"
#include "er_shade.h"
#include "er_stream.h"
#include "er_ring.h"

using namespace erd;

#ifdef ER_TIME_PROBE
#define ER_TPS(n)                                                                                       \
    {                                                                                                    \
        const unsigned long long tp_now = __builtin_amdgcn_s_memtime();                                  \
        if (tp_sec < 10u && (threadIdx.x & 63) == 0) atomicAdd(&s_tp[tp_sec], (unsigned)((tp_now - tp_last) >> 4)); \
        tp_last = tp_now;                                                                                \
        tp_sec = (n);                                                                                    \
    }
#undef ER_TP
#define ER_TP(n) ER_TPS(n)
#else
#define ER_TPS(n) ((void)0)
#endif
// ... 672 lines not shown
                    ER_SP(W.stamp(slot) = sp_now();)
                } else {
                    push_closest = true;
                }
                push_shadow = pending;
                push_light = EXT && lpending;
                if (alive) {
                    if (!fin_next) {
                        W.ray_o(slot) = make_float4(ray.o.x, ray.o.y, ray.o.z, MESH ? mesh_d : 0.0f);
                        W.ray_d(slot) = make_float4(ray.d.x, ray.d.y, ray.d.z, EXT ? prev_pdf : -1.0f);
                    }
                    W.light(slot) = make_float4(light.x, light.y, light.z, __builtin_bit_cast(float, rs));
                    W.reduc(slot) = make_float4(reduction.x, reduction.y, reduction.z,
                                                __builtin_bit_cast(float, bounce | (pending ? WF_PENDING_BIT : 0u) | ((EXT && lpending) ? WF_LPENDING_BIT : 0u)));
                    s_wait[ls] = (push_closest ? 1u : 0u) + (push_shadow ? 1u : 0u) + (push_light ? 1u : 0u) + (fin_next ? ST_FIN : 0u);
                }
                if (SPEC) {
                    cancel = cancel_w == (uint32_t)SP_INVALID;
                    if (!cancel) {
                        const unsigned long long add = (unsigned long long)(t_bounce | (t_shaded << 10) | (t_hdri << 20)) |
                                                       ((unsigned long long)((push_closest ? 1u : 0u) + (push_shadow ? 1u : 0u) + (push_light ? 1u : 0u)) << 32);
                        __hip_atomic_fetch_add((unsigned long long*)&W.tally_a(slot), add, __ATOMIC_RELAXED, __HIP_MEMORY_SCOPE_WORKGROUP);
                        if (COUNT) {
                            W.tally_tex(slot) += t_texels;
                            atomicAdd(&W.tally_nodes(slot), t_nodes);
                            atomicAdd(&W.tally_tris(slot), t_tris);
                        }
                    } else {
                        push_closest = false; push_shadow = false; push_light = false; to_finish = false;
                        retire = true;
                    }
                }
            }
            if (!fin_mode) {
                if (__ballot(to_finish)) {
                    __builtin_amdgcn_fence(__ATOMIC_RELEASE, "workgroup");
                    st_push<ST_SQ_LOG2>(s_fq, s_fq_ctl, to_finish, ls, status, ST_ERR_SHADE);
                }
            } else if (have && !parked && !discard) {
                ER_TPS(6);
                const uint32_t pxy = W.pix(slot);
                const uint32_t idx = st_pixel_index(S, pxy);
                const float4 L4 = W.light(slot);
                F3 light = f3(L4.x, L4.y, L4.z);
                rs = __builtin_bit_cast(uint32_t, L4.w);
                const float4 R4 = W.reduc(slot);
                const uint32_t packed = __builtin_bit_cast(uint32_t, R4.w);
                if (S.tile_cost) __hip_atomic_fetch_add(&S.tile_cost[(pxy >> 19) * S.tiles_x + ((pxy & 0xFFFFu) >> 3)], (packed & 0xFFFFu) + 1u, __ATOMIC_RELAXED, __HIP_MEMORY_SCOPE_AGENT);
                if ((e >> ST_SLOT_BITS) != 0) {
                    F3 reduction = f3(R4.x, R4.y, R4.z);
                    uint32_t bounce = packed & 0xFFFFu;
                    if (packed & WF_PENDING_BIT) {
                        const float4 c = W.occluded(slot) ? W.c_occ(slot) : W.c_vis(slot);
                        light = light + f3(c.x, c.y, c.z);
                    }
                    if (EXT && (packed & WF_LPENDING_BIT)) {
                        const uint32_t q = slot + W.slots;
                        const float4 c = W.occluded(q) ? W.c_occ(q) : W.c_vis(q);
                        light = light + f3(c.x, c.y, c.z);
                    }
                    const float4 d = W.ray_d(slot);
                    Ray ray;
                    ray.o = f3s(0);
                    ray.d = f3(d.x, d.y, d.z);
                    float prev_pdf = EXT ? d.w : -1.0f;
                    float mesh_d = 0.0f;
                    const int hslot = -1;
                    bool done = false, pending = false, lpending = false;
                    c_bounce++;
#define ER_BOUNCE_HDRI_QUERY(sr, self_slot, d_self, cv, co) ((void)(sr), (void)(self_slot), (void)(d_self), (void)(cv), (void)(co))
#define ER_BOUNCE_LIGHT_QUERY(lr, self_slot, limit, lv, lo) ((void)(lr), (void)(self_slot), (void)(limit), (void)(lv), (void)(lo))
#define ER_BOUNCE_FIRST_HIT(n, t, b) ((void)(n), (void)(t), (void)(b))
#include "er_bounce.inc"
#undef ER_BOUNCE_HDRI_QUERY
#undef ER_BOUNCE_LIGHT_QUERY
#undef ER_BOUNCE_FIRST_HIT
                    (void)bounce; (void)done; (void)pending; (void)lpending; (void)prev_pdf; (void)mesh_d;
                }
                const float4 an = W.aov_n(slot), at = W.aov_t(slot), ab = W.aov_b(slot);
                const uint32_t sa = S.samples[idx];
                const uint32_t sa2 = accumulate_sample(S, idx, sa, light, f3(an.x, an.y, an.z), f3(at.x, at.y, at.z), f3(ab.x, ab.y, ab.z));
                if (sa2 != sa) S.samples[idx] = sa2;
                S.rng[idx] = rs;
                c_paths++;
                if (SPEC) {
                    const uint32_t ta = W.tally_a(slot);
                    c_bounce += ta & 0x3FFu; c_shaded += (ta >> 10) & 0x3FFu; c_hdri += (ta >> 20) & 0x3FFu;
                    c_rays += W.tally_rays(slot);
                    if (COUNT) { c_texels += W.tally_tex(slot); c_nodes += W.tally_nodes(slot); c_tris += W.tally_tris(slot); }
                }
                if (SPEC && spec_on) {
                    {
                        const uint32_t ta = W.tally_a(slot);
                        const uint32_t per_opaque = MESH ? 7u : (EXT && (S.ext_flags & ER_FLAG_POINT_LIGHTS) != 0 && S.light_count > 0) ? 5u : 4u;
                        uint32_t nd = 5u + ((ta >> 10) & 0x3FFu) + per_opaque * ((ta >> 20) & 0x3FFu);
                        nd = nd > ST_DRAWS_MASK ? 0u : nd;
                        const uint32_t oldh = S.px_draws[idx];
                        uint32_t cand = oldh & ST_DRAWS_MASK, conf = (oldh >> ST_CONF_SHIFT) & 7u;
                        if (nd != 0u && nd == cand) conf = conf < 7u ? conf + 1u : 7u;
                        else if (conf >= 2u) conf -= 2u;
                        else { cand = nd; conf = nd != 0u ? 1u : 0u; }
                        uint32_t maj = (oldh >> ST_MAJ_SHIFT) & ST_DRAWS_MASK, votes = (oldh >> ST_VOTE_SHIFT) & 7u, mean16 = oldh >> ST_LONG_SHIFT;
                        if (nd != 0u && nd == maj) votes = votes < 7u ? votes + 1u : 7u;
                        else if (votes > 0u) votes--;
                        else { maj = nd; votes = nd != 0u ? 1u : 0u; }
                        const uint32_t its16 = ((ta & 0x3FFu) + ((e >> ST_SLOT_BITS) != 0 ? 1u : 0u)) << 4;
                        mean16 = (uint32_t)((int)mean16 + (((int)(its16 > 511u ? 511u : its16) - (int)mean16) >> 3));
                        S.px_draws[idx] = cand | (conf << ST_CONF_SHIFT) | (votes << ST_VOTE_SHIFT) | (maj << ST_MAJ_SHIFT) | (mean16 << ST_LONG_SHIFT);
                    }
                    const uint32_t link = W.spec_link(slot);
                    if (link) {
                        const uint32_t f = g0 + link - 1u;
                        const bool ok = W.spec_start(f) == rs;
                        __builtin_amdgcn_fence(__ATOMIC_RELEASE, "workgroup");
                        const uint32_t old = atomicExch(&W.spec_word(f), ok ? (uint32_t)SP_VALID : (uint32_t)SP_INVALID);
                        atomicAdd(&s_spec[ok ? 1 : 2], 1u);
                        if (old == (uint32_t)SP_PARKED) {
                            __builtin_amdgcn_fence(__ATOMIC_ACQUIRE, "workgroup");
                            wake = true;
                            wake_entry = W.spec_entry(f);
                        }
                        has_spec = ok;
                    }
                }
                ER_SP(sSS += sp_now() - W.stamp0(slot); sNS++;)
                left_after = W.left(slot) - 1;
                done_idx = pxy;
                want_pixel = true;
                if (KEEP && spec_keep != 0u) {
                    const uint32_t front = atomicMin(&s_front, left_after);
                    keep_own = left_after > 0u && !has_spec && left_after >= front + spec_keep;
                }
            }
            ER_MARK("shader_pixel_ring");
            ER_TPS(7);
            if (__ballot(want_pixel)) {
                const bool back = want_pixel && left_after > 0 && !has_spec && !(KEEP && keep_own);
                const unsigned long long mb = __ballot(back);
                if (mb) {
                    __builtin_amdgcn_fence(__ATOMIC_RELEASE, "workgroup");
                    uint32_t base = 0;
                    if (lane == 0) base = er_ring_reserve(s_px_ctl, (uint32_t)__popcll(mb));
                    base = (uint32_t)__builtin_amdgcn_readlane((int)base, 0);
                    if (back) {
                        const uint32_t pos = base + (uint32_t)__popcll(mb & below), cell = pos & (ring_cap - 1u);
                        if (!er_bits_acquire(s_pxbits, cell)) atomicOr(status, ST_ERR_PIXEL);
                        ring[cell] = make_uint2(done_idx, left_after | ST_LAP_TAG(pos, ring_cap));
                    }
                    __builtin_amdgcn_fence(__ATOMIC_RELEASE, "workgroup");
                    if (lane == 0) er_ring_publish(s_px_ctl, (uint32_t)__popcll(mb));
                }
                bool spawn_want = false;
                uint32_t spawn_rs = 0, spawn_pxy = 0, spawn_left = 0, spawn_draws = 0;
                const bool want_take = want_pixel && !(KEEP && keep_own);
                const unsigned long long mw = __ballot(want_take);
                uint32_t hb2 = 0;
                const uint32_t granted2 = st_take(s_px_ctl, (uint32_t)__popcll(mw), hb2, er_ring_peek(s_px_ctl));
                const uint32_t rank = (uint32_t)__popcll(mw & below);
                if (want_take && rank < granted2) {
                    const uint32_t ppos = hb2 + rank, pcell = ppos & (ring_cap - 1u);
                    const unsigned long long* cell = (const unsigned long long*)(ring + pcell);
                    const uint32_t want_tag = ST_LAP_TAG(ppos, ring_cap);
                    unsigned long long w = 0;
                    uint32_t y = 0, guard = 0;
                    while (true) {
                        w = __hip_atomic_load(cell, __ATOMIC_RELAXED, __HIP_MEMORY_SCOPE_WORKGROUP);
                        y = (uint32_t)(w >> 32);
                        if ((y & ~ST_LEFT_MASK) == want_tag) break;
                        if (++guard >= ER_RING_GUARD) { y = 0; break; }
                        __builtin_amdgcn_s_sleep(1);
                    }
                    __builtin_amdgcn_fence(__ATOMIC_ACQUIRE, "workgroup");
                    er_bits_release(s_pxbits, pcell);
                    const uint32_t nidx = (uint32_t)w;
                    y &= ST_LEFT_MASK;
                    if (y != 0) {
                        spawn_rs = st_begin_sample<SPEC>(S, W, slot, nidx, y);
                        if (SPEC && spec_on && y > 1u) {
                            const uint32_t h = S.px_draws[st_pixel_index(S, nidx)];
                            const bool longp = spec_long != 0u && (h >> ST_LONG_SHIFT) >= spec_long;
                            const bool sure = ((h >> ST_CONF_SHIFT) & 7u) >= spec_need;
                            spawn_draws = (longp && !sure) ? ((h >> ST_MAJ_SHIFT) & ST_DRAWS_MASK) : (h & ST_DRAWS_MASK);
                            spawn_want = spawn_draws != 0u && (longp || sure) && waited >= spec_slack;
                        }
                        spawn_pxy = nidx; spawn_left = y - 1u;
                        s_wait[ls] = 1u;
                        push_closest = true;
                    } else {
                        atomicOr(status, ST_ERR_PIXEL);
                        retire = true;
                    }
                } else if (want_take) {
                    retire = true;
                }
                if (KEEP && keep_own) {
                    spawn_rs = st_begin_sample<SPEC>(S, W, slot, done_idx, left_after);
                    if (SPEC && spec_on && left_after > 1u) {
                        const uint32_t h = S.px_draws[st_pixel_index(S, done_idx)];
                        const bool longp = spec_long != 0u && (h >> ST_LONG_SHIFT) >= spec_long;
                        const bool sure = ((h >> ST_CONF_SHIFT) & 7u) >= spec_need;
                        spawn_draws = (longp && !sure) ? ((h >> ST_MAJ_SHIFT) & ST_DRAWS_MASK) : (h & ST_DRAWS_MASK);
                        spawn_want = spawn_draws != 0u && (longp || sure) && waited >= spec_slack;
                    }
                    spawn_pxy = done_idx; spawn_left = left_after - 1u;
                    s_wait[ls] = 1u;
                    push_closest = true;
                }
                if (SPEC && spec_on && __ballot(spawn_want)) {
                    const unsigned long long msp = __ballot(spawn_want);
                    uint32_t hbf = 0;
                    const uint32_t gf = st_take(s_free_ctl, (uint32_t)__popcll(msp), hbf, er_ring_peek(s_free_ctl));
                    const uint32_t rk = (uint32_t)__popcll(msp & below);
                    uint32_t fslot = 0;
                    bool got_free = false;
                    if (spawn_want && rk < gf) {
                        got_free = er_ring_get(s_free, ST_SQ_LOG2, hbf + rk, fslot);
                        if (!got_free) atomicOr(status, ST_ERR_SHADE);
                    }
                    __builtin_amdgcn_fence(__ATOMIC_ACQUIRE, "workgroup");
                    if (got_free) {
                        uint32_t sp = spawn_rs;
                        for (uint32_t k = 0; k < spawn_draws; k++) { sp ^= sp << 13; sp ^= sp >> 17; sp ^= sp << 5; }
                        st_begin_sample<SPEC>(S, W, g0 + fslot, spawn_pxy, spawn_left, true, sp);
                        W.spec_link(slot) = fslot + 1u;
                        s_wait[fslot] = 1u;
                        push_spec = true;
                        ls_spec = fslot;
                    }
                    const unsigned long long mgot = __ballot(got_free);
                    if (mgot && lane == (int)(__ffsll((long long)mgot) - 1)) {
                        atomicAdd(&s_ctl[C_LIVE], (uint32_t)__popcll(mgot));
                        atomicAdd(&s_spec[0], (uint32_t)__popcll(mgot));
                    }
                }
            }
            if (SPEC && spec_on && __ballot(wake)) {
                __builtin_amdgcn_fence(__ATOMIC_RELEASE, "workgroup");
                st_push<ST_SQ_LOG2>(s_fq, s_fq_ctl, wake, wake_entry, status, ST_ERR_SHADE);
            }
            ER_MARK("shader_publish");
            ER_TPS(8);
            __builtin_amdgcn_fence(__ATOMIC_RELEASE, "workgroup");
            {
                const unsigned long long mc = __ballot(push_closest), ms = __ballot(push_shadow), ml = EXT ? __ballot(push_light) : 0ull;
                const unsigned long long mx = SPEC ? __ballot(push_spec) : 0ull;
                const unsigned nc = (unsigned)__popcll(mc), ns = (unsigned)__popcll(ms), nl = (unsigned)__popcll(ml) + (unsigned)__popcll(mx);
                ER_SP(if (push_closest) { const uint32_t spF = sp_now(); sEF += spF - spE; W.stamp(slot) = spF; })
                if (nc + ns + nl) {
                    uint32_t base = 0;
                    if (lane == 0) base = er_ring_reserve(s_rq_ctl, nc + ns + nl);
                    base = (uint32_t)__builtin_amdgcn_readlane((int)base, 0);
                    bool ok = true;
                    if (push_closest) ok = er_ring_put(s_rq, RQ_LOG2, base + (uint32_t)__popcll(mc & below), ls) && ok;
                    if (push_shadow) ok = er_ring_put(s_rq, RQ_LOG2, base + nc + (uint32_t)__popcll(ms & below), ls | (1u << ST_SLOT_BITS)) && ok;
                    if (EXT && push_light) ok = er_ring_put(s_rq, RQ_LOG2, base + nc + ns + (uint32_t)__popcll(ml & below), ls | (2u << ST_SLOT_BITS)) && ok;
                    if (SPEC && push_spec) ok = er_ring_put(s_rq, RQ_LOG2, base + nc + ns + (uint32_t)__popcll(ml) + (uint32_t)__popcll(mx & below), ls_spec) && ok;
                    if (!ok) atomicOr(status, ST_ERR_RAY);
                    if (lane == 0) er_ring_publish(s_rq_ctl, nc + ns + nl);
                }
                const unsigned long long mr = __ballot(retire);
                if (SPEC && spec_on && mr) st_push<ST_SQ_LOG2>(s_free, s_free_ctl, retire, ls, status, ST_ERR_SHADE);
                if (mr) {
                    const uint32_t nr = (uint32_t)__popcll(mr);
                    if (lane == 0) {
                        const uint32_t oldl = atomicSub(&s_ctl[C_LIVE], nr);
                        if (oldl == nr) s_ctl[C_DONE] = 1;
                    }
                }
            }
            have = false;
            ER_TPS(9);
#ifdef ER_TIME_PROBE
            if (lane == 0) { atomicAdd(&s_tp[10], 1u); atomicAdd(&s_tp[11], granted); }
#endif
        }
        ER_MARK("shader_loop_end");
        ER_SP({ unsigned long long* spc = (unsigned long long*)&S.counters->node_visits; sp_add(spc + 3, sDE); sp_add(spc + 4, sEF); sp_add(spc + 6, sGE); sp_add(spc + 7, sNG); sp_add(spc + 8, sSS); atomicAdd(&S.counters->paths, (unsigned long long)sNS); })
    }
    ER_MARK("epilogue");
#if defined(ER_STAGE_PROBE) || defined(ER_TRACER_PROBE)
    return;
#endif
#ifdef ER_TIME_PROBE
    __syncthreads();
    if (threadIdx.x == 0) {
        unsigned long long* c = (unsigned long long*)&S.counters->node_visits;
        for (int i = 1; i < 10; i++) atomicAdd(&c[i - 1], (unsigned long long)s_tp[i]);
        atomicAdd(&S.counters->paths, (unsigned long long)s_tp[10]);
        atomicAdd(&S.counters->bounce_samples, (unsigned long long)s_tp[11]);
        atomicAdd(&S.counters->rays, (unsigned long long)s_tp[12]);
    }
    return;
#endif
    if (SPEC) {
        if (lane == 0) {
            const unsigned q0 = atomicExch(&s_spec[0], 0u), q1 = atomicExch(&s_spec[1], 0u), q2 = atomicExch(&s_spec[2], 0u);
            if (q0 | q1 | q2) { atomicAdd(status + ER_SC_SPEC, q0); atomicAdd(status + ER_SC_SPEC + 1, q1); atomicAdd(status + ER_SC_SPEC + 2, q2); }
        }
    }
    unsigned t0 = st_wave_sum(c_paths), t1 = st_wave_sum(c_bounce), t2 = st_wave_sum(c_rays), t3 = st_wave_sum(c_shaded), t4 = st_wave_sum(c_hdri);
    unsigned t5 = 0, t6 = 0, t7 = 0;
    if (COUNT) { t5 = st_wave_sum(c_nodes); t6 = st_wave_sum(c_tris); t7 = st_wave_sum(c_texels); }
    if (lane == 0) {
        atomicMax((unsigned long long*)(status + ER_SC_END + 2 * (blockIdx.x & 7u)), (unsigned long long)wall_clock64());
        if (t0) atomicAdd(&S.counters->paths, (unsigned long long)t0);
        if (t1) atomicAdd(&S.counters->bounce_samples, (unsigned long long)t1);
        if (t2) atomicAdd(&S.counters->rays, (unsigned long long)t2);
        if (t3) atomicAdd(&S.counters->shaded_hits, (unsigned long long)t3);
        if (t4) atomicAdd(&S.counters->hdri_samples, (unsigned long long)t4);
        if (COUNT) {
            atomicAdd(&S.counters->node_visits, (unsigned long long)t5);
            atomicAdd(&S.counters->tri_tests, (unsigned long long)t6);
            atomicAdd(&S.counters->texel_fetches, (unsigned long long)t7);
            atomicAdd(&S.counters->trace_wave_steps, (unsigned long long)c_wsteps);
            atomicAdd(&S.counters->trace_busy_lanes, (unsigned long long)c_busy);
            atomicAdd(&S.counters->trace_node_lanes, (unsigned long long)c_nl);
            atomicAdd(&S.counters->trace_tri_lanes, (unsigned long long)c_tl);
        }
    }
}

#ifndef ER_STREAM_MESH_TU
hipError_t er_probe_stream(const char** which) {
    hipFuncAttributes a;
    *which = "er_stream_kernel";
    hipError_t e = hipFuncGetAttributes(&a, (const void*)er_stream_kernel<false, false, false, 1024u, false, 0>);
    if (e == hipSuccess) e = hipFuncGetAttributes(&a, (const void*)er_stream_kernel<false, false, false, 768u, true, 0>);
    return e != hipSuccess ? e : hipFuncGetAttributes(&a, (const void*)er_stream_kernel<false, false, false, 768u, true, 2>);
}

ErStreamLaunchForm er_stream_launch_form(uint32_t max_bounces, uint32_t tri_count, uint32_t waves, bool spec, bool keep) {
    static const uint32_t spec_flag = [] {
        const char* e = getenv("ER_STREAM_SPEC");
        const char* b = getenv("ER_STREAM_SPEC_SLACK");
        int v = e ? atoi(e) : 2, bl = b ? atoi(b) : 1;
        return ((uint32_t)(v < 0 ? 0 : (v > 7 ? 7 : v)) << 8) | ((uint32_t)(bl < 0 ? 0 : (bl > 255 ? 255 : bl)) << 12);
    }();
    static const uint32_t spec_long16 = [] {
        const char* e = getenv("ER_STREAM_SPEC_LONG");
        int v = e ? atoi(e) : ER_STREAM_SPEC_LONG_DEFAULT;
        return (uint32_t)(v < 0 ? 0 : (v > 16 ? 16 : v));
    }();
    static const uint32_t spec_keep = [] {
        const char* e = getenv("ER_STREAM_SPEC_KEEP");
        int v = e ? atoi(e) : ER_STREAM_SPEC_KEEP_DEFAULT;
        return (uint32_t)(v < 0 ? 0 : (v > 7 ? 7 : v));
    }();
    waves = waves == 12u ? 12u : 16u;
    const uint32_t long_thr = waves == 12u ? max_bounces * spec_long16 : 0u;
    const uint32_t spec_now = (max_bounces <= 1000u && tri_count >= ER_STREAM_SPEC_MIN_TRIS) ? (spec_flag | ((long_thr > 511u ? 0u : long_thr) << 20) | (((waves == 16u && keep) ? spec_keep : 0u) << 29)) : 0u;
    const uint32_t keep_plain = (keep && waves == 16u) ? (spec_keep << 29) : 0u;
    if (spec && spec_now) return {2u, waves, spec_now};
    if (keep_plain) return {1u, waves, keep_plain};
    return {0u, waves, 0u};
}

#endif

#ifdef ER_STREAM_MESH_TU
#define ER_STREAM_LAUNCH er_launch_stream_mesh
#else
#define ER_STREAM_LAUNCH er_launch_stream
#endif
void ER_STREAM_LAUNCH(const ErStreamLaunch& L) {
    const DevScene& S = *L.S;
#ifndef ER_STREAM_MESH_TU
    if (er_mesh_active(S)) {
        er_launch_stream_mesh(L);
        return;
    }
#endif
    static const uint32_t refill_min = [] {
        const char* e = getenv("ER_STREAM_REFILL_MIN");
        int v = e ? atoi(e) : 12;
        return (uint32_t)(v < 1 ? 1 : (v > 64 ? 64 : v));
    }();
    static const uint32_t batch_min = [] {
        const char* e = getenv("ER_STREAM_BATCH_MIN");
        int v = e ? atoi(e) : 64;
        const char* p = getenv("ER_STREAM_BATCH_SPINS");
        int sp = p ? atoi(p) : 3;
        return (uint32_t)(v < 1 ? 1 : (v > 64 ? 64 : v)) | ((uint32_t)(sp < 0 ? 0 : (sp > 100000 ? 100000 : sp)) << 8);
    }();
    static const uint32_t fin_min = [] {
        const char* e = getenv("ER_STREAM_FIN_MIN");
        int v = e ? atoi(e) : 64;
        return (uint32_t)(v < 1 ? 1 : (v > 64 ? 64 : v));
    }();
    if (S.owned_tile_count == 0 || L.n_samples == 0) return;
    const ErStreamLaunchForm form = er_stream_launch_form(S.max_bounces, S.tri_count, L.waves, L.spec, L.keep);
    const uint32_t waves = form.waves, last = fin_min | form.bits;
    const bool count = L.count;
    uint32_t tracers = L.tracers;
    if (tracers > ST_MAX_TRACERS) tracers = ST_MAX_TRACERS;
    if (tracers > waves - 1u) tracers = waves - 1u;
    if (tracers < 1u) tracers = 1u;
    const bool fuse = S.fused_any != 0u;
    auto pick = [&](auto with, auto without) { return fuse ? with : without; };
#ifdef ER_STREAM_MESH_TU
#define ST_PICK(THREADS, SPECV)                                                                                                                                  \
    (count ? pick(er_stream_kernel<true, true, true, THREADS, true, SPECV>, er_stream_kernel<true, true, true, THREADS, false, SPECV>)                           \
           : pick(er_stream_kernel<false, true, true, THREADS, true, SPECV>, er_stream_kernel<false, true, true, THREADS, false, SPECV>))
#else
    const bool ext = er_ext_active(S);
#define ST_PICK(THREADS, SPECV)                                                                                                                                  \
    (count ? (ext ? pick(er_stream_kernel<true, true, false, THREADS, true, SPECV>, er_stream_kernel<true, true, false, THREADS, false, SPECV>)                   \
                  : pick(er_stream_kernel<true, false, false, THREADS, true, SPECV>, er_stream_kernel<true, false, false, THREADS, false, SPECV>))                 \
           : (ext ? pick(er_stream_kernel<false, true, false, THREADS, true, SPECV>, er_stream_kernel<false, true, false, THREADS, false, SPECV>)                 \
                  : pick(er_stream_kernel<false, false, false, THREADS, true, SPECV>, er_stream_kernel<false, false, false, THREADS, false, SPECV>)))
#endif
    auto k16 = ST_PICK(1024u, 0);
    auto k16k = ST_PICK(1024u, 1);
    auto k16s = ST_PICK(1024u, 2);
    auto k12s = ST_PICK(768u, 2);
    auto k12 = ST_PICK(768u, 0);
#undef ST_PICK
    StState st;
    st.base = (char*)L.records;
    st.spill = (uint2*)L.spill;
    st.slots = L.slots;
    st.stride = er_stream_record_bytes(L.lights);
    const DevScene __attribute__((address_space(4)))* dS = (const DevScene __attribute__((address_space(4)))*)L.S_dev;
    auto go = [&](auto kernel) {
        hipLaunchKernelGGL(kernel, dim3(L.blocks), dim3(waves * 64u), 0, L.stream, dS, st, L.deal, L.deal_count, (uint2*)L.ring, L.ring_cap, L.status, L.n_samples, tracers, refill_min, batch_min, last);
    };
    if (waves == 12u) { if (form.form == 2u) go(k12s); else go(k12); }
    else if (form.form == 2u) go(k16s);
    else if (form.form == 1u) go(k16k);
    else go(k16);
}

#undef ER_STREAM_LAUNCH

#ifndef ER_STREAM_MESH_TU
uint32_t er_stream_record_bytes(bool lights) { return lights ? ST_STRIDE_LIGHTS : ST_STRIDE_PLAIN; }
size_t er_stream_spill_entries(uint32_t blocks) { return (size_t)blocks * 16 * ER_SPILL_PER_WAVE; }
#endif
```

elevenrender_amd/csrc/er_stream_host.cpp:

```cpp
#include <algorithm>
#include <map>

#include "er_scene.h"
#include "../../include/eleven_hip_debug.h"

using namespace erh;

uint32_t er_stream_deal_tiles(const uint32_t* owned, uint32_t count, uint32_t tiles_x, uint32_t blocks, bool xcd_aware, std::vector<uint32_t>& out, uint32_t edge) {
    if (edge == 0u) {
        const char* e = getenv("ER_STREAM_SUPER_TILE");
        const int v = e ? atoi(e) : 0;
        edge = v >= 1 ? (uint32_t)v : ER_STREAM_SUPER_TILE_DEFAULT;
    }
    const uint32_t X = (xcd_aware && blocks % 8u == 0u) ? 8u : 1u, per = blocks / X, S8 = edge;
    const uint32_t super_x = (tiles_x + S8 - 1u) / S8;
    std::map<uint32_t, std::vector<uint32_t>> by_super;
    for (uint32_t i = 0; i < count; i++) {
        const uint32_t tx = owned[i] % tiles_x, ty = owned[i] / tiles_x;
        by_super[X == 1u ? 0u : (ty / S8) * super_x + tx / S8].push_back(owned[i]);
    }
    std::vector<std::vector<uint32_t>> seq(X);
    for (auto& kv : by_super) {
        uint32_t best = 0;
        for (uint32_t x = 1; x < X; x++) if (seq[x].size() < seq[best].size()) best = x;
        seq[best].insert(seq[best].end(), kv.second.begin(), kv.second.end());
    }
    const char* lv = getenv("ER_STREAM_LEVEL_XCDS");
    for (; !(lv && atoi(lv) == 0);) {
        uint32_t hi = 0, lo = 0;
        for (uint32_t x = 1; x < X; x++) {
            if (seq[x].size() > seq[hi].size()) hi = x;
            if (seq[x].size() < seq[lo].size()) lo = x;
        }
        const size_t diff = seq[hi].size() - seq[lo].size();
        if (diff <= 1u) break;
        const size_t n = diff / 2u;
        seq[lo].insert(seq[lo].end(), seq[hi].end() - (ptrdiff_t)n, seq[hi].end());
        seq[hi].resize(seq[hi].size() - n);
    }
    uint32_t maxk = 0;
    for (uint32_t x = 0; x < X; x++) maxk = std::max<uint32_t>(maxk, (uint32_t)((seq[x].size() + per - 1u) / per));
    out.assign((size_t)blocks * maxk, 0xFFFFFFFFu);
    for (uint32_t x = 0; x < X; x++)
        for (size_t sidx = 0; sidx < seq[x].size(); sidx++) {
            const uint32_t j = (uint32_t)(sidx % per), k = (uint32_t)(sidx / per), b = j * X + x;
            out[(size_t)b + (size_t)k * blocks] = seq[x][sidx];
        }
    return maxk;
}

bool stream_xcd_aware(size_t owned_tiles, uint32_t blocks) {
    const char* xe = getenv("ER_STREAM_XCD_TILES");
    return xe ? atoi(xe) != 0 : owned_tiles * 64 > (size_t)blocks * ER_STREAM_SLOTS;
}

StreamDeal stream_deal_owned(const std::vector<uint32_t>& owned, uint32_t tiles_x, uint32_t cus) {
    StreamDeal d;
    d.most = er_stream_deal_tiles(owned.data(), (uint32_t)owned.size(), tiles_x, cus, stream_xcd_aware(owned.size(), cus), d.tiles);
    return d;
}

StreamForm stream_choose_form(size_t tiles, uint32_t blocks, bool light_query, uint32_t tri_count, uint32_t flags) {
    StreamForm f;
    const uint32_t large_tracers = (light_query || tri_count > 4000000u) ? 12u : 13u;
    f.tracers = large_tracers;
    f.waves = 16;
    const size_t px_per_cu = tiles * 64 / std::max<uint32_t>(1u, blocks);
    const uint32_t small_tracers = px_per_cu > ER_STREAM_TEN_TRACERS_SHARE ? 10u : 9u;
    if (px_per_cu <= ER_STREAM_SMALL_SHARE) { f.waves = 12; f.tracers = small_tracers; }
    f.adapt = px_per_cu >= 4u * ER_STREAM_SLOTS && !(flags & ER_FLAG_COUNTERS);
    f.keep = px_per_cu <= ER_STREAM_KEEP_SHARE;
    f.spec = px_per_cu <= ER_STREAM_SPEC_SHARE;
    if (const char* e = getenv("ER_STREAM_SPEC_FORM")) f.spec = atoi(e) != 0;
    if (const char* e = getenv("ER_STREAM_KEEP")) f.keep = atoi(e) != 0;
    if (const char* e = getenv("ER_STREAM_WAVES")) { f.waves = atoi(e) == 12 ? 12 : 16; f.tracers = f.waves == 12 ? small_tracers : large_tracers; }
    if (const char* e = getenv("ER_STREAM_TRACERS")) { f.tracers = (uint32_t)std::min(13, std::max(1, atoi(e))); f.adapt = false; }
    if (const char* e = getenv("ER_STREAM_ADAPT")) f.adapt = atoi(e) != 0;
    return f;
}

static void stream_set_form(ErScene* s, size_t tiles) {
    StreamHost& st = s->st;
    st.form = stream_choose_form(tiles, st.blocks, st.lights, s->tri_count, s->params.flags);
    st.tracers_start = st.form.tracers; st.low_streak = 0; st.up_budget = 1;
}

static hipError_t stream_drop_pending_deal(ErScene* s) {
    s->st.deal_pending = false;
    s->dev.tile_cost = s->ad_dev.tile_cost = nullptr;
    s->st.deal_large.clear(); s->st.deal_large.shrink_to_fit();
    return hipMemcpyAsync(s->d_dev.p, &s->dev, sizeof(DevScene), hipMemcpyHostToDevice, s->stream);
}

int stream_begin(ErScene* s, const std::vector<uint32_t>& owned, StreamDeal& deal, uint32_t cus, bool light_query) {
    StreamHost& st = s->st;
    int rc;
    st.blocks = cus;
    st.lights = light_query;
    stream_set_form(s, owned.size());
    st.readings = 0;
    const size_t slots = (size_t)st.blocks * ER_STREAM_SLOTS, npx = (size_t)s->x_res * s->y_res;
    if ((rc = upload(s->d_wf4, nullptr, slots * er_stream_record_bytes(light_query) / sizeof(float4), s->stream)) != ER_OK) return rc;
    if ((rc = upload(s->d_wf1, nullptr, ER_STREAM_CTL_LEAD + ER_SC_WORDS, s->stream)) != ER_OK) return rc;
    if ((rc = upload(s->d_spill, nullptr, er_stream_spill_entries(st.blocks), s->stream)) != ER_OK) return rc;
    st.ctl = s->d_wf1.p;
    HIP_TRY(hipMemsetAsync(st.ctl, 0, (ER_STREAM_CTL_LEAD + ER_SC_WORDS) * sizeof(uint32_t), s->stream));
    st.spec[0] = st.spec[1] = st.spec[2] = 0;
    const bool xcd_aware = stream_xcd_aware(owned.size(), st.blocks);
    const uint32_t tiles_x = s->tiles_x();
    uint32_t most = deal.most;
    st.deal_off = 0; st.deal_n = (uint32_t)deal.tiles.size();
    st.deal_alt_off = 0; st.deal_alt_n = 0;
    st.xcd_spread = -1.0;
    const char* adapt_knob = getenv("ER_STREAM_ADAPT");
    st.deal_pending = false;
    st.deal_large.clear();
    st.d_tile_cost.release();
    if (xcd_aware && st.blocks % 8u == 0u && owned.size() * 64 / st.blocks >= ER_STREAM_SLOTS * 3u / 2u && !(s->params.flags & ER_FLAG_COUNTERS) &&
        !getenv("ER_STREAM_SUPER_TILE") && !(adapt_knob && atoi(adapt_knob) == 0)) {
        std::vector<uint32_t> large;
        const uint32_t most_large = er_stream_deal_tiles(owned.data(), (uint32_t)owned.size(), tiles_x, st.blocks, xcd_aware, large, ER_STREAM_SUPER_TILE_LARGE);
        if ((size_t)most_large * 64u <= ER_STREAM_MAX_RING) {
            st.deal_alt_off = (uint32_t)deal.tiles.size(); st.deal_alt_n = (uint32_t)large.size();
            deal.tiles.insert(deal.tiles.end(), large.begin(), large.end());
            most = std::max(most, most_large);
            st.deal_large.swap(large);
            const size_t n_tiles = (size_t)tiles_x * s->tiles_y();
            if ((rc = upload(st.d_tile_cost, nullptr, n_tiles, s->stream)) != ER_OK) return rc;
            HIP_TRY(hipMemsetAsync(st.d_tile_cost.p, 0, n_tiles * sizeof(uint32_t), s->stream));
            st.deal_pending = true;
        }
    }
    if ((rc = upload(st.d_px_draws, nullptr, npx, s->stream)) != ER_OK) return rc;
    HIP_TRY(hipMemsetAsync(st.d_px_draws.p, 0, npx * sizeof(uint32_t), s->stream));
    if ((rc = upload(st.d_deal, deal.tiles.data(), deal.tiles.size(), s->stream)) != ER_OK) return rc;
    if (s->x_res > 65535u || s->y_res > 65535u)
        return fail(ER_ERR_INVALID_ARG, "er_render_begin: ER_FLAG_STREAM carries a pixel as x | y << 16: frames up to 65535 x 65535; use ER_FLAG_WAVEFRONT (the automatic choice does)");
    st.ring_cap = 64u;
    while (st.ring_cap < most * 64u) st.ring_cap <<= 1;
    if (st.ring_cap > ER_STREAM_MAX_RING)
        return fail(ER_ERR_INVALID_ARG, "er_render_begin: ER_FLAG_STREAM serves at most " + std::to_string((size_t)ER_STREAM_MAX_RING * st.blocks) +
                                            " owned pixels per rank; use ER_FLAG_WAVEFRONT (the automatic choice does)");
    if ((rc = upload(st.d_ticket, nullptr, (size_t)st.blocks * (size_t)st.ring_cap * 2, s->stream)) != ER_OK) return rc;
    return ER_OK;
}

int stream_redeal(ErScene* s) {
    StreamHost& st = s->st;
    const bool large = st.large_deal_in_use();
    if (st.deal_pending) HIP_TRY(stream_drop_pending_deal(s));
    const uint32_t count = (uint32_t)s->ad_active.size(), tiles_x = s->tiles_x();
    std::vector<uint32_t> deal;
    uint32_t most = er_stream_deal_tiles(s->ad_active.data(), count, tiles_x, st.blocks, stream_xcd_aware(count, st.blocks), deal, large ? ER_STREAM_SUPER_TILE_LARGE : 0u);
    if ((size_t)most * 64u > st.ring_cap) most = er_stream_deal_tiles(s->ad_active.data(), count, tiles_x, st.blocks, false, deal);
    if ((size_t)most * 64u > st.ring_cap) return fail(ER_ERR_STATE, "er_render_samples: the active tiles do not fit the pixel rings");
    int rc;
    if ((rc = upload(st.d_deal, deal.data(), deal.size(), s->stream)) != ER_OK) return rc;
    st.deal_off = 0; st.deal_n = (uint32_t)deal.size();
    st.deal_alt_off = 0; st.deal_alt_n = 0;
    stream_set_form(s, count);
    HIP_TRY(hipStreamSynchronize(s->stream));
    return ER_OK;
}

static int stream_launch(ErScene* s, uint32_t k) {
    StreamHost& st = s->st;
    HIP_TRY(hipMemsetAsync(st.status() + ER_SC_ITERS, 0, (ER_SC_WORDS - ER_SC_ITERS) * sizeof(uint32_t), s->stream));
    HIP_TRY(hipMemsetAsync(st.status() + ER_SC_START, 0xFF, 2 * sizeof(uint32_t), s->stream));
    if (k > 0) st.launches++;
    ErStreamLaunch L;
    L.S = &s->dev; L.S_dev = s->d_dev.p;
    L.records = s->d_wf4.p; L.slots = st.blocks * ER_STREAM_SLOTS; L.lights = st.lights;
    L.spill = s->d_spill.p;
    L.deal = st.d_deal.p + st.deal_off; L.deal_count = st.deal_n;
    L.ring = st.d_ticket.p; L.ring_cap = st.ring_cap;
    L.status = st.status();
    L.n_samples = k;
    L.count = (s->params.flags & ER_FLAG_COUNTERS) != 0;
    L.blocks = st.blocks; L.tracers = st.form.tracers; L.waves = st.form.waves; L.spec = st.form.spec; L.keep = st.form.keep;
    L.stream = s->stream;
    er_launch_stream(L);
    return ER_OK;
}

int stream_enqueue(ErScene* s, uint32_t n) {
    StreamHost& st = s->st;
    static const bool split_first = [] { const char* e = getenv("ER_STREAM_SPLIT_FIRST"); return !(e && atoi(e) == 0); }();
    int rc;
    if (st.deal_pending && n >= 2u && split_first) {
        if ((rc = stream_launch(s, 1u)) != ER_OK) return rc;
        HIP_TRY(hipGetLastError());
        HIP_TRY(hipStreamSynchronize(s->stream));
        if ((rc = er_scene_stream_status(s, "er_render_samples")) != ER_OK) return rc;
        st.probe_launch = true;
        stream_adapt(s);
        st.probe_launch = false;
        n -= 1u;
    }
    return stream_launch(s, n);
}

int er_scene_stream_status(ErScene* s, const char* who) {
    StreamHost& st = s->st;
    if (!(s->params.flags & ER_FLAG_STREAM) || !st.ctl) return ER_OK;
    uint32_t w[ER_SC_WORDS] = {0};
    HIP_TRY(hipMemcpy(w, st.status(), sizeof(w), hipMemcpyDeviceToHost));
    if (st.spec_seen != st.launches) {
        st.spec_seen = st.launches;
        for (int k = 0; k < 3; k++) st.spec[k] += w[ER_SC_SPEC + k];
    }
    if (w[ER_SC_STATUS] != 0)
        return fail(ER_ERR_STATE, std::string(who) + ": the streaming schedule stopped without finishing (watchdog status " + std::to_string(w[ER_SC_STATUS]) + "); the planes are incomplete");
    auto u64 = [&](uint32_t i) { return (unsigned long long)w[i] | ((unsigned long long)w[i + 1] << 32); };
    const unsigned long long iters = u64(ER_SC_ITERS), busy = u64(ER_SC_BUSY);
    st.busy = iters ? (double)busy / (64.0 * (double)iters) : 0.0;
    const unsigned long long t0 = u64(ER_SC_START);
    unsigned long long lo = ~0ull, hi = 0;
    for (uint32_t x = 0; x < 8; x++) { const unsigned long long e = u64(ER_SC_END + 2 * x); lo = std::min(lo, e); hi = std::max(hi, e); }
    st.xcd_spread = (t0 != ~0ull && lo > t0 && hi - t0 >= 200000ull) ? (double)(hi - lo) / (double)(hi - t0) : -1.0;
    st.launch_ms = (t0 != ~0ull && hi > t0) ? (double)(hi - t0) * 1e-5 : 0.0;
    return ER_OK;
}

void stream_adapt(ErScene* s) {
    StreamHost& st = s->st;
    if (!(s->params.flags & ER_FLAG_STREAM)) return;
    const bool verbose = getenv("ER_STREAM_VERBOSE") != nullptr;
    if (st.adapted == st.launches) return;
    st.adapted = st.launches;
    if (verbose && !st.form.adapt) fprintf(stderr, "[er_stream] tracer lanes %.3f full at %u + %u waves (fixed split)\n", st.busy, st.form.tracers, st.form.waves - st.form.tracers);
    if (st.deal_pending) {
        std::vector<uint32_t> cost(st.d_tile_cost.n);
        if (hipMemcpy(cost.data(), st.d_tile_cost.p, cost.size() * sizeof(uint32_t), hipMemcpyDeviceToHost) == hipSuccess) {
            double x[8] = {0, 0, 0, 0, 0, 0, 0, 0};
            const std::vector<uint32_t>& L = st.deal_large;
            for (size_t i = 0; i < L.size(); i++)
                if (L[i] != 0xFFFFFFFFu && L[i] < cost.size()) x[(i % st.blocks) % 8u] += (double)cost[L[i]];
            double lo = x[0], hi = x[0], sum = 0;
            for (double v : x) { lo = std::min(lo, v); hi = std::max(hi, v); sum += v; }
            const double spread = sum > 0 ? (hi - lo) / (sum / 8.0) : 0.0;
            const char* lim_env = getenv("ER_STREAM_COST_SPREAD_MAX");
            const double limit = lim_env ? atof(lim_env) : (double)ER_STREAM_COST_SPREAD_MAX;
            const bool take = sum > 0 && spread <= limit;
            st.cost_spread = spread;
            if (verbose) fprintf(stderr, "[er_stream] counted work of the XCDs' shares on super-tiles of %u: %.4f of the mean apart (limit %.4f) -> %s\n", (unsigned)ER_STREAM_SUPER_TILE_LARGE, spread,
                                 limit, take ? "large regions" : "the default deal stays");
            if (take) { st.deal_off = st.deal_alt_off; st.deal_n = st.deal_alt_n; }
        }
        (void)stream_drop_pending_deal(s);
        (void)hipStreamSynchronize(s->stream);
    }
    if (verbose && st.xcd_spread >= 0.0)
        fprintf(stderr, "[er_stream] XCDs finished %.3f of the launch apart (a measured time: printed, nothing is decided on it)\n", st.xcd_spread);
    if (!st.form.adapt || st.busy <= 0.0 || st.probe_launch) return;
    const uint32_t lo = st.form.waves == 12 ? 7u : 10u;
    const uint32_t before = st.form.tracers;
    const char* forced = getenv("ER_STREAM_FORCE_BUSY");
    double busy = st.busy;
    if (forced) {
        const char* q = forced;
        for (uint32_t k = 0; k < st.readings; k++) { const char* c = strchr(q, ','); if (!c) break; q = c + 1; }
        busy = atof(q);
    }
    st.readings++;
    if (!forced && st.launch_ms < ER_STREAM_ADAPT_MIN_MS) {
        if (verbose) fprintf(stderr, "[er_stream] tracer lanes %.3f full in a launch of %.2f ms: too short to be a reading\n", st.busy, st.launch_ms);
        return;
    }
    if (busy < 0.85) {
        if (++st.low_streak >= 2u && st.form.tracers > lo) { st.form.tracers--; st.low_streak = 0; }
    } else {
        st.low_streak = 0;
        if (busy > 0.93 && st.up_budget > 0u && st.form.tracers < st.tracers_start) { st.form.tracers++; st.up_budget--; }
    }
    if (verbose) fprintf(stderr, "[er_stream] tracer lanes %.3f full%s at %u + %u waves -> %u + %u\n", busy, forced ? " (forced reading)" : "", before, st.form.waves - before, st.form.tracers, st.form.waves - st.form.tracers);
}

void stream_fill_info(const ErScene* s, ErStreamInfo* out) {
    const StreamHost& st = s->st;
    out->waves = st.form.waves; out->tracers = st.form.tracers;
    out->large_regions = st.large_deal_in_use() ? 1u : 0u;
    out->deal_pending = st.deal_pending ? 1u : 0u;
    out->launches = (uint32_t)st.launches;
    out->pixels_per_cu = (uint32_t)((size_t)s->dev.owned_tile_count * 64 / std::max<uint32_t>(1u, st.blocks));
    out->lanes_busy = st.busy; out->launch_ms = st.launch_ms; out->cost_spread = st.cost_spread;
    out->spec_started = st.spec[0]; out->spec_right = st.spec[1]; out->spec_wrong = st.spec[2];
    out->form = er_stream_launch_form(s->dev.max_bounces, s->tri_count, st.form.waves, st.form.spec, st.form.keep).form;
}
```

elevenrender_amd/csrc/er_stream_host.h:

```cpp
#pragma once
#include <stdint.h>

#include <vector>

#include "er_devbuf.h"
#include "er_stream.h"

struct ErScene;
struct ErStreamInfo;

struct StreamForm {
    uint32_t waves = 16, tracers = 0;
    bool adapt = false, keep = false, spec = false;
};
StreamForm stream_choose_form(size_t tiles, uint32_t blocks, bool light_query, uint32_t tri_count, uint32_t flags);
bool stream_xcd_aware(size_t owned_tiles, uint32_t blocks);

struct StreamDeal {
    std::vector<uint32_t> tiles;
    uint32_t most = 0;
};
StreamDeal stream_deal_owned(const std::vector<uint32_t>& owned, uint32_t tiles_x, uint32_t cus);

struct StreamHost {
    uint32_t blocks = 0;
    uint32_t ring_cap = 0;
    bool lights = false;
    StreamForm form;
    uint32_t tracers_start = 0;
    uint32_t low_streak = 0;
    uint32_t up_budget = 1;
    uint32_t readings = 0;
    uint32_t* ctl = nullptr;
    uint32_t* status() const { return ctl + ER_STREAM_CTL_LEAD; }
    double busy = 0.0;
    double launch_ms = 0.0;
    double xcd_spread = 0.0;
    double cost_spread = -1.0;
    uint64_t spec[3] = {0, 0, 0};
    uint64_t spec_seen = 0;
    uint64_t launches = 0, adapted = 0;
    bool probe_launch = false;
    erh::DevBuf<uint32_t> d_deal, d_ticket;
    uint32_t deal_off = 0, deal_n = 0;
    uint32_t deal_alt_off = 0, deal_alt_n = 0;
    bool deal_pending = false;
    erh::DevBuf<uint32_t> d_tile_cost;
    std::vector<uint32_t> deal_large;
    erh::DevBuf<uint32_t> d_px_draws;

    bool large_deal_in_use() const { return deal_alt_n != 0u && deal_off == deal_alt_off; }
    void release() {
        d_deal.release(); d_ticket.release(); d_tile_cost.release(); d_px_draws.release();
        ctl = nullptr;
    }
};

int stream_begin(ErScene* s, const std::vector<uint32_t>& owned, StreamDeal& deal, uint32_t cus, bool light_query);
int stream_redeal(ErScene* s);
int stream_enqueue(ErScene* s, uint32_t n);
void stream_adapt(ErScene* s);
void stream_fill_info(const ErScene* s, ErStreamInfo* out);
```

elevenrender_amd/render.py:

```python
import ctypes as C
from dataclasses import dataclass

import numpy as np

from . import abi


@dataclass
class RenderParameters:
    width: int = 1280
    height: int = 720
    sampleTarget: int = 100
    denoise: bool = False
    device: str = ""
    block_size: int = 8
    max_bounces: int = 5
    rank: int = 0
    world: int = 1
    flags: int = 0


@dataclass
class RenderInfo:
    samples: int = 0


def list_devices():
    lib = abi.load()
    out = []
    for i in range(lib.er_device_count()):
        info = abi.ErDeviceInfo()
        abi.check(lib.er_device_info(i, C.byref(info)))
        out.append({"name": info.name.decode(), "platform": info.platform.decode(),
                    "memory": int(info.memory_bytes), "max_compute_units": int(info.compute_units),
                    "is_compatible": bool(info.compatible), "online_compiler": False, "type": "gpu",
                    "arch": info.arch.decode()})
    return out


def measure_hbm_peak(device=0, nbytes=0, iters=0):
    lib = abi.load()
    a, b = C.c_float(), C.c_float()
    abi.check(lib.er_measure_hbm_peak(device, nbytes, iters, C.byref(a), C.byref(b)))
    return a.value, b.value


class RenderingManager:

    def __init__(self, pars: RenderParameters = None):
        self.pars = pars or RenderParameters()
        self.lib = abi.load()
        self.handle = C.c_void_p()
        self.scene = None

    def start_rendering(self, scene: abi.SceneData):
        self.close()
        self.scene = scene
        self.pars.width, self.pars.height = scene.x_res, scene.y_res
        abi.check(self.lib.er_scene_create(C.byref(scene.desc()), C.byref(self.handle)))
        dev = 0
        sel = self.pars.device
        if sel.startswith("hip:"):
            dev = int(sel[4:])
        elif sel:
            dev = self.lib.er_device_find(sel.encode())
            if dev < 0:
                abi.check(dev)
        p = abi.ErRenderParams(self.pars.sampleTarget, self.pars.block_size, self.pars.max_bounces, dev,
                               self.pars.rank, self.pars.world, self.pars.flags)
        abi.check(self.lib.er_render_begin(self.handle, C.byref(p)))

    def render(self, n_samples, blocking=True):
        if blocking:
            abi.check(self.lib.er_render_samples(self.handle, n_samples))
        else:
            abi.check(self.lib.er_render_samples_async(self.handle, n_samples))

    def wait(self):
        ms = C.c_float()
        abi.check(self.lib.er_wait(self.handle, C.byref(ms)))
        return ms.value

    def get_pass(self, name="beauty"):
        p = abi.PASS_NAMES.get(str(name).lower(), abi.PASS_BEAUTY)
        out = np.empty((self.scene.y_res, self.scene.x_res, 4), np.float32)
        abi.check(self.lib.er_read_pass(self.handle, p, out.ctypes.data_as(C.POINTER(C.c_float))))
        return out

    def get_render_info(self):
        v = C.c_uint32()
        abi.check(self.lib.er_samples_done(self.handle, C.byref(v)))
        return RenderInfo(samples=v.value)

    def set_adaptive(self, threshold, min_samples=0, interval=0):
        p = None if threshold is None else C.byref(abi.ErAdaptiveParams(threshold, min_samples, interval))
        abi.check(self.lib.er_adaptive_set(self.handle, p))

    def adaptive_info(self):
        a = abi.ErAdaptiveInfo()
        abi.check(self.lib.er_adaptive_info(self.handle, C.byref(a)))
        return {n: getattr(a, n) for n, _ in abi.ErAdaptiveInfo._fields_}

    def light_info(self):
        li = abi.ErLightInfo()
        abi.check(self.lib.er_light_info(self.handle, C.byref(li)))
        return {n: getattr(li, n) for n, _ in abi.ErLightInfo._fields_}

    def debug_light_table(self):
        n = self.light_info()["emitters"]
        tri = np.zeros(n, np.int32)
        cdf = np.zeros(n, np.float32)
        if n:
            abi.check(self.lib.er_debug_read_light_table(self.handle, tri.ctypes.data_as(C.POINTER(C.c_int32)), cdf.ctypes.data_as(C.POINTER(C.c_float)), n))
        return tri, cdf

    def tile_state(self):
        tx, ty = (self.scene.x_res + 7) // 8, (self.scene.y_res + 7) // 8
        err = np.empty((ty, tx), np.float32)
        spp = np.empty((ty, tx), np.uint32)
        abi.check(self.lib.er_read_tile_state(self.handle, err.ctypes.data_as(C.POINTER(C.c_float)), spp.ctypes.data_as(C.POINTER(C.c_uint32))))
        return err, spp

    def denoise(self, levels=0, colour_sigma=0.0):
        abi.check(self.lib.er_denoise(self.handle, levels, colour_sigma))

    def read_samples(self):
        out = np.empty(self.scene.x_res * self.scene.y_res, np.uint32)
        abi.check(self.lib.er_read_samples(self.handle, out.ctypes.data_as(C.POINTER(C.c_uint32))))
        return out

    def read_rng(self):
        out = np.empty(self.scene.x_res * self.scene.y_res, np.uint32)
        abi.check(self.lib.er_read_rng(self.handle, out.ctypes.data_as(C.POINTER(C.c_uint32))))
        return out

    def counters(self):
        c = abi.ErCounters()
        abi.check(self.lib.er_get_counters(self.handle, C.byref(c)))
        return {n: int(getattr(c, n)) for n, _ in abi.ErCounters._fields_}

    def profile(self):
        pr = abi.ErProfile()
        abi.check(self.lib.er_get_profile(self.handle, C.byref(pr)))
        return {n: getattr(pr, n) for n, _ in abi.ErProfile._fields_}

    def stream_info(self):
        si = abi.ErStreamInfo()
        abi.check(self.lib.er_debug_stream_info(self.handle, C.byref(si)))
        return {n: getattr(si, n) for n, _ in abi.ErStreamInfo._fields_}

    def accel_info(self):
        a = abi.ErAccelInfo()
        abi.check(self.lib.er_accel_info(self.handle, C.byref(a)))
        return {n: getattr(a, n) for n, _ in abi.ErAccelInfo._fields_}

    def debug_read_accel(self):
        info = abi.ErAccelDump()
        abi.check(self.lib.er_debug_read_accel(self.handle, C.byref(info), None, 0, None, 0, None, 0, None, 0))
        nodes = np.zeros(info.node_count, abi.NODE_DTYPE)
        raw8 = np.zeros((info.node8_count, info.node8_pieces * 16), np.uint8)
        isect = np.zeros(info.tri_count + 1, abi.ISECT_DTYPE)
        attr = np.zeros(info.tri_count, abi.attr_dtype(info.attr_pieces))
        vp = lambda a: a.ctypes.data_as(C.c_void_p)
        abi.check(self.lib.er_debug_read_accel(self.handle, C.byref(info), vp(nodes), nodes.nbytes, vp(raw8), raw8.nbytes, vp(isect), isect.nbytes,
                                               vp(attr), attr.nbytes))
        nodes8 = np.ascontiguousarray(raw8[:, :abi.NODE8_DTYPE.itemsize]).view(abi.NODE8_DTYPE).reshape(-1)
        return abi.accel_dump_dict(info, nodes=nodes, nodes8=nodes8, isect=isect, attr=attr, node8_stride_tail=raw8[:, abi.NODE8_DTYPE.itemsize:])

    def debug_closest_hit(self, origins, dirs):
        o = np.ascontiguousarray(origins, np.float32).reshape(-1, 3)
        d = np.ascontiguousarray(dirs, np.float32).reshape(-1, 3)
        n = len(o)
        tri = np.empty(n, np.int32)
        pos = np.empty((n, 3), np.float32)
        dist = np.empty(n, np.float32)
        fp = lambda a: a.ctypes.data_as(C.POINTER(C.c_float))
        abi.check(self.lib.er_debug_closest_hit(self.handle, fp(o), fp(d), n, tri.ctypes.data_as(C.POINTER(C.c_int32)), fp(pos), fp(dist)))
        return tri, pos, dist

    def debug_trace_rays(self, origins, dirs, self_slots=None, limits=None):
        o = np.ascontiguousarray(origins, np.float32).reshape(-1, 3)
        d = np.ascontiguousarray(dirs, np.float32).reshape(-1, 3)
        n = len(o)
        tri, slot, info = np.empty(n, np.int32), np.empty(n, np.int32), np.empty(n, np.int32)
        pos, dist = np.empty((n, 3), np.float32), np.empty(n, np.float32)
        fp = lambda a: a.ctypes.data_as(C.POINTER(C.c_float))
        ip = lambda a: a.ctypes.data_as(C.POINTER(C.c_int32))
        if self_slots is None:
            abi.check(self.lib.er_debug_trace_rays(self.handle, fp(o), fp(d), n, None, None, ip(tri), ip(slot), fp(pos), fp(dist), ip(info)))
            return tri, slot, pos, dist, info
        ss = np.ascontiguousarray(self_slots, np.int32)
        lim = np.ascontiguousarray(limits, np.float32)
        abi.check(self.lib.er_debug_trace_rays(self.handle, fp(o), fp(d), n, ip(ss), fp(lim), ip(tri), ip(slot), fp(pos), fp(dist), ip(info)))
        return tri.astype(bool), info

    def debug_eval(self, kind, items, out_width):
        a = np.ascontiguousarray(items, np.float32)
        out = np.zeros((a.shape[0], out_width), np.float32)
        fp = lambda x: x.ctypes.data_as(C.POINTER(C.c_float))
        abi.check(self.lib.er_debug_eval(self.handle, kind, fp(a), a.shape[0], a.shape[1], fp(out), out_width))
        return out

    def debug_trace_pixel(self, idx, max_recs=64):
        recs = (abi.ErTraceRec * max_recs)()
        n = C.c_int()
        abi.check(self.lib.er_debug_trace_pixel(self.handle, idx, recs, max_recs, C.byref(n)))
        return [recs[i] for i in range(n.value)]

    def state_export(self):
        n = C.c_uint64()
        abi.check(self.lib.er_state_size(self.handle, C.byref(n)))
        buf = np.empty(n.value, np.uint8)
        abi.check(self.lib.er_state_export(self.handle, buf.ctypes.data_as(C.c_void_p), n.value))
        return buf

    def state_import(self, buf):
        b = np.ascontiguousarray(buf, np.uint8)
        abi.check(self.lib.er_state_import(self.handle, b.ctypes.data_as(C.c_void_p), b.size))

    def owned_count(self, rank):
        v = C.c_uint64()
        abi.check(self.lib.er_owned_count(self.handle, rank, C.byref(v)))
        return int(v.value)

    def pack_owned(self, pass_id, dev_ptr):
        abi.check(self.lib.er_pack_owned(self.handle, pass_id, C.c_void_p(dev_ptr)))

    def unpack_owned(self, pass_id, src_rank, dev_ptr):
        abi.check(self.lib.er_unpack_owned(self.handle, pass_id, src_rank, C.c_void_p(dev_ptr)))

    def close(self):
        if self.handle:
            self.lib.er_scene_destroy(self.handle)
            self.handle = C.c_void_p()

    def __del__(self):
        try:
            self.close()
        except Exception:
            pass
```

include/eleven_hip_debug.h:

```cpp
#ifndef ELEVEN_HIP_DEBUG_H
#define ELEVEN_HIP_DEBUG_H
#include <stdint.h>
#ifdef __cplusplus
extern "C" {
#endif

typedef struct ErBvhCheck {
    uint32_t node_count, leaf_count, max_depth, max_leaf_size;
    uint32_t tris_in_leaves;
    uint32_t duplicate_tris;
    uint32_t uncontained;
    uint32_t unreachable_nodes;
    float lift_bound;
    float build_ms;
    double sah_cost;
} ErBvhCheck;

int er_debug_bvh_check(const float* vertices, const float* normals, uint32_t tri_count, int threads, ErBvhCheck* out);

typedef struct ErAccelDump {
    uint32_t tri_count;
    uint32_t node_count;
    uint32_t node8_count;
    uint32_t node8_pieces;
    uint32_t attr_pieces;
    uint32_t max_depth;
    uint32_t max_depth8;
    uint32_t builder;
    float lo[3], hi[3];
    float lift_bound;
    float max_lift;
} ErAccelDump;

struct ErScene;
int er_debug_read_accel(struct ErScene* scene, ErAccelDump* info, void* nodes, uint64_t nodes_cap, void* nodes8, uint64_t nodes8_cap,
                        void* isect, uint64_t isect_cap, void* attr, uint64_t attr_cap);

int er_debug_bvh_dump(const float* vertices, const float* normals, uint32_t tri_count, int threads, ErAccelDump* info, void* nodes, uint64_t nodes_cap,
                      void* nodes8, uint64_t nodes8_cap, uint32_t* slot_to_tri, uint64_t slot_cap, float* tri_lift, uint64_t lift_cap);

int er_debug_cdf_search(const float* cdf, int length, const float* values, int32_t* out, int count);

struct ErScene;
int er_debug_closest_hit(struct ErScene* scene, const float* origins, const float* dirs, uint32_t n, int32_t* tri_ids, float* positions, float* distances);

int er_debug_trace_rays(struct ErScene* scene, const float* origins, const float* dirs, uint32_t n, const int32_t* self_slots,
                        const float* limits, int32_t* tri_ids, int32_t* slots, float* positions, float* distances, int32_t* info);

typedef struct ErTraceRec {
    int32_t bounce;
    int32_t tri;
    int32_t shadow_tri;
    int32_t opaque;
    float position[3];
    float wi[3];
    float light[3];
    float reduction[3];
    int32_t shadow_occ;
    int32_t light_occ;
} ErTraceRec;

int er_debug_trace_pixel(struct ErScene* scene, uint32_t idx, ErTraceRec* recs, int max_recs, int* count);

int er_debug_read_light_table(struct ErScene* scene, int32_t* tri_index, float* cdf, uint32_t cap);

enum { ER_FN_RNG = 0, ER_FN_CAMERA_RAY, ER_FN_TRI_HIT, ER_FN_DISNEY_EVAL, ER_FN_DISNEY_PDF, ER_FN_DISNEY_SAMPLE, ER_FN_SPHERICAL,
       ER_FN_REV_SPHERICAL, ER_FN_TEXTURE, ER_FN_HDRI_SEARCH, ER_FN_HDRI_PDF, ER_FN_MATH, ER_FN_COUNT };
int er_debug_eval(struct ErScene* scene, int kind, const float* in, uint32_t n, uint32_t in_stride, float* out, uint32_t out_stride);

struct ErComm;
int er_debug_comm_create_local(uint32_t world, struct ErComm** out);

typedef struct ErStreamInfo {
    uint32_t waves, tracers;
    uint32_t large_regions;
    uint32_t deal_pending;
    uint32_t launches;
    uint32_t pixels_per_cu;
    double lanes_busy;
    double launch_ms;
    double cost_spread;
    uint64_t spec_started, spec_right, spec_wrong;
    uint32_t form;
    uint32_t reserved;
} ErStreamInfo;
int er_debug_stream_info(struct ErScene* s, ErStreamInfo* out);

int er_debug_gather_buffers(struct ErScene* s, uint32_t peer, void** in_ptr, uint64_t* in_bytes, void** mine_ptr, uint64_t* mine_bytes);

int er_debug_comm_loopback(struct ErComm* c, uint64_t bytes, double* ms);

int er_debug_stream_deal(const uint32_t* owned, uint32_t count, uint32_t tiles_x, uint32_t blocks, int xcd_aware, uint32_t edge, uint32_t* out, uint32_t out_cap,
                         uint32_t* most);

typedef struct ErStreamForm {
    uint32_t waves, tracers;
    uint32_t adapt;
    uint32_t keep, spec;
    uint32_t reserved;
} ErStreamForm;
int er_debug_stream_form(uint32_t tiles, uint32_t blocks, int light_query, uint32_t tri_count, uint32_t flags, ErStreamForm* out);

void er_debug_set_host_alloc_limit(uint64_t bytes);

void er_debug_set_gpu_build_failure(int kind);

#ifdef __cplusplus
}
#endif
#endif
```

Baseline: 2025 Msamples/s.

## Level the stream tile deal across workgroups by counted per-tile cost

After the first counted launch, the host reads back per-tile work counts and redistributes tiles between XCD groups and then across workgroups within each XCD. It uses greedy longest-first assignment under the ring capacity cap and uploads the levelled deal into a reserved region of the deal buffer. This targets the idle tail where some workgroups finish much later than others. It also records per-workgroup end timestamps for diagnostics. It adds a host-side sort and rebalance plus an extra sync, keeps cost counting active during the probe launch, and changes the tile order each workgroup sees, which may hurt locality.

```diff
diff --git a/elevenrender_amd/abi.py b/elevenrender_amd/abi.py
--- a/elevenrender_amd/abi.py
+++ b/elevenrender_amd/abi.py
@@ -107,6 +107,11 @@
                 ("pixels_per_cu", C.c_uint32), ("lanes_busy", C.c_double), ("launch_ms", C.c_double), ("cost_spread", C.c_double),
                 ("spec_started", C.c_uint64), ("spec_right", C.c_uint64), ("spec_wrong", C.c_uint64),
                 ("form", C.c_uint32), ("reserved", C.c_uint32)]
+
+
+class ErStreamBalance(C.Structure):
+    _fields_ = [("blocks", C.c_uint32), ("most", C.c_uint32), ("levelled", C.c_uint32), ("counting", C.c_uint32), ("cost_tiles", C.c_uint32), ("cap", C.c_uint32),
+                ("launch_ticks", C.c_uint64)]
 
 
 class ErStreamForm(C.Structure):
@@ -229,6 +234,10 @@
 
 OPTIONAL_SYMBOLS = {
     "er_debug_stream_form": (C.c_int, [C.c_uint32, C.c_uint32, C.c_int, C.c_uint32, C.c_uint32, C.POINTER(ErStreamForm)]),
+    "er_debug_stream_level": (C.c_int, [C.POINTER(C.c_uint32), C.c_uint32, C.c_uint32, C.c_uint32, C.POINTER(C.c_uint32), C.c_uint32, C.c_uint32, C.POINTER(C.c_uint32),
+                                        C.c_uint32, C.POINTER(C.c_uint32)]),
+    "er_debug_stream_balance": (C.c_int, [_P, C.POINTER(ErStreamBalance), C.POINTER(C.c_uint64), C.POINTER(C.c_uint32), C.POINTER(C.c_uint64), C.c_uint32, C.POINTER(C.c_uint32),
+                                          C.c_uint32, C.POINTER(C.c_uint32), C.c_uint32]),
     "er_debug_read_accel": (C.c_int, [_P, C.POINTER(ErAccelDump), _P, C.c_uint64, _P, C.c_uint64, _P, C.c_uint64, _P, C.c_uint64]),
     "er_debug_bvh_dump": (C.c_int, [_FP, _FP, C.c_uint32, C.c_int, C.POINTER(ErAccelDump), _P, C.c_uint64, _P, C.c_uint64, C.POINTER(C.c_uint32), C.c_uint64,
                                     _FP, C.c_uint64]),
diff --git a/elevenrender_amd/csrc/er_api.cpp b/elevenrender_amd/csrc/er_api.cpp
--- a/elevenrender_amd/csrc/er_api.cpp
+++ b/elevenrender_amd/csrc/er_api.cpp
@@ -536,7 +536,7 @@
     D.owned_tiles = s->d_owned.p;
     D.owned_tile_count = owned_tiles;
     D.counters = s->d_counters.p;
-    D.tile_cost = ((s->params.flags & ER_FLAG_STREAM) && s->st.deal_pending) ? s->st.d_tile_cost.p : nullptr;
+    D.tile_cost = ((s->params.flags & ER_FLAG_STREAM) && s->st.counting) ? s->st.d_tile_cost.p : nullptr;
     D.px_draws = (s->params.flags & ER_FLAG_STREAM) ? s->st.d_px_draws.p : nullptr;
     {
         const erd::CamTrig t = erd::camera_trig(D.cam);
diff --git a/elevenrender_amd/csrc/er_debug_api.cpp b/elevenrender_amd/csrc/er_debug_api.cpp
--- a/elevenrender_amd/csrc/er_debug_api.cpp
+++ b/elevenrender_amd/csrc/er_debug_api.cpp
@@ -42,6 +42,44 @@
     *most = er_stream_deal_tiles(owned, count, tiles_x, blocks, xcd_aware != 0, deal, edge);
     if (deal.size() > out_cap || (deal.size() && !out)) return fail(ER_ERR_INVALID_ARG, "er_debug_stream_deal: out holds fewer than blocks * most entries");
     for (size_t i = 0; i < deal.size(); i++) out[i] = deal[i];
+    return ER_OK;
+}
+
+static int er_debug_stream_level_impl(const uint32_t* deal, uint32_t deal_n, uint32_t tiles_x, uint32_t blocks, const uint32_t* cost, uint32_t cost_n, uint32_t cap, uint32_t* out,
+                                      uint32_t out_cap, uint32_t* most) {
+    if ((deal_n && !deal) || (cost_n && !cost) || !tiles_x || !blocks || deal_n % blocks != 0u || !cap || !most) return fail(ER_ERR_INVALID_ARG, "er_debug_stream_level: bad argument");
+    std::vector<uint32_t> lvl;
+    *most = er_stream_level_by_cost(std::vector<uint32_t>(deal, deal + deal_n), tiles_x, blocks, cost, cost_n, cap, lvl);
+    if (lvl.size() > out_cap || (lvl.size() && !out)) return fail(ER_ERR_INVALID_ARG, "er_debug_stream_level: out holds fewer than blocks * most entries");
+    for (size_t i = 0; i < lvl.size(); i++) out[i] = lvl[i];
+    return ER_OK;
+}
+
+static int er_debug_stream_balance_impl(ErScene* s, ErStreamBalance* info, uint64_t* wg_ticks, uint32_t* wg_tiles, uint64_t* wg_cost, uint32_t wg_cap, uint32_t* deal, uint32_t deal_cap,
+                                        uint32_t* tile_cost, uint32_t cost_cap) {
+    if (!s || !info) return fail(ER_ERR_INVALID_ARG, "er_debug_stream_balance: NULL argument");
+    std::lock_guard<std::mutex> lk(s->mtx);
+    memset(info, 0, sizeof(*info));
+    if (!s->begun || !(s->params.flags & ER_FLAG_STREAM)) return ER_OK;
+    const StreamHost& st = s->st;
+    info->blocks = st.blocks;
+    info->most = st.blocks ? (uint32_t)(st.deal_host.size() / st.blocks) : 0u;
+    info->levelled = st.deal_levelled ? 1u : 0u;
+    info->counting = st.counting ? 1u : 0u;
+    info->cost_tiles = (uint32_t)st.cost_host.size();
+    info->cap = st.ring_cap / 64u;
+    info->launch_ticks = st.launch_end > st.launch_start ? st.launch_end - st.launch_start : 0u;
+    if (wg_cap >= st.blocks) {
+        std::vector<uint32_t> tiles; std::vector<uint64_t> cost, ticks;
+        stream_balance(s, tiles, cost, ticks);
+        for (uint32_t b = 0; b < st.blocks; b++) {
+            if (wg_ticks) wg_ticks[b] = ticks[b];
+            if (wg_tiles) wg_tiles[b] = tiles[b];
+            if (wg_cost) wg_cost[b] = cost[b];
+        }
+    }
+    if (deal && deal_cap >= st.deal_host.size()) for (size_t i = 0; i < st.deal_host.size(); i++) deal[i] = st.deal_host[i];
+    if (tile_cost && cost_cap >= st.cost_host.size()) for (size_t i = 0; i < st.cost_host.size(); i++) tile_cost[i] = st.cost_host[i];
     return ER_OK;
 }
 
@@ -362,6 +400,12 @@
 int er_debug_stream_deal(const uint32_t* owned, uint32_t count, uint32_t tiles_x, uint32_t blocks, int xcd_aware, uint32_t edge, uint32_t* out, uint32_t out_cap, uint32_t* most) {
     return guarded("er_debug_stream_deal", [&]() -> int { return er_debug_stream_deal_impl(owned, count, tiles_x, blocks, xcd_aware, edge, out, out_cap, most); });
 }
+int er_debug_stream_level(const uint32_t* deal, uint32_t deal_n, uint32_t tiles_x, uint32_t blocks, const uint32_t* cost, uint32_t cost_n, uint32_t cap, uint32_t* out, uint32_t out_cap, uint32_t* most) {
+    return guarded("er_debug_stream_level", [&]() -> int { return er_debug_stream_level_impl(deal, deal_n, tiles_x, blocks, cost, cost_n, cap, out, out_cap, most); });
+}
+int er_debug_stream_balance(ErScene* s, ErStreamBalance* info, uint64_t* wg_ticks, uint32_t* wg_tiles, uint64_t* wg_cost, uint32_t wg_cap, uint32_t* deal, uint32_t deal_cap, uint32_t* tile_cost, uint32_t cost_cap) {
+    return guarded("er_debug_stream_balance", [&]() -> int { return er_debug_stream_balance_impl(s, info, wg_ticks, wg_tiles, wg_cost, wg_cap, deal, deal_cap, tile_cost, cost_cap); });
+}
 int er_debug_stream_form(uint32_t tiles, uint32_t blocks, int light_query, uint32_t tri_count, uint32_t flags, ErStreamForm* out) {
     return guarded("er_debug_stream_form", [&]() -> int { return er_debug_stream_form_impl(tiles, blocks, light_query, tri_count, flags, out); });
 }
diff --git a/elevenrender_amd/csrc/er_stream.h b/elevenrender_amd/csrc/er_stream.h
--- a/elevenrender_amd/csrc/er_stream.h
+++ b/elevenrender_amd/csrc/er_stream.h
@@ -53,10 +53,13 @@
     ER_SC_START = 5,
     ER_SC_END = 7,
     ER_SC_SPEC = 23,
-    ER_SC_WORDS = 26
+    ER_SC_WORDS = 26,
+    ER_SC_WG_END = 27
 };
 constexpr uint32_t ER_STREAM_CTL_LEAD = 1;
-static_assert((ER_STREAM_CTL_LEAD + ER_SC_ITERS) % 2u == 0u && ER_SC_BUSY % 2u == 1u && ER_SC_START % 2u == 1u && ER_SC_END % 2u == 1u, "the 64-bit control words are 8-byte aligned");
+static_assert((ER_STREAM_CTL_LEAD + ER_SC_ITERS) % 2u == 0u && ER_SC_BUSY % 2u == 1u && ER_SC_START % 2u == 1u && ER_SC_END % 2u == 1u && ER_SC_WG_END % 2u == 1u && ER_SC_WG_END >= ER_SC_WORDS,
+              "the 64-bit control words are 8-byte aligned");
+constexpr uint32_t er_stream_ctl_words(uint32_t blocks) { return ER_SC_WG_END + 2u * blocks; }
 
 struct ErStreamLaunch {
     const DevScene* S = nullptr;
@@ -84,6 +87,7 @@
 struct ErStreamLaunchForm { uint32_t form, waves, bits; };
 ErStreamLaunchForm er_stream_launch_form(uint32_t max_bounces, uint32_t tri_count, uint32_t waves, bool spec, bool keep);
 uint32_t er_stream_deal_tiles(const uint32_t* owned, uint32_t count, uint32_t tiles_x, uint32_t blocks, bool xcd_aware, std::vector<uint32_t>& out, uint32_t edge = 0);
+uint32_t er_stream_level_by_cost(const std::vector<uint32_t>& deal, uint32_t tiles_x, uint32_t blocks, const uint32_t* cost, size_t cost_n, uint32_t cap, std::vector<uint32_t>& out);
 uint32_t er_stream_record_bytes(bool lights);
 size_t er_stream_spill_entries(uint32_t blocks);
 hipError_t er_probe_stream(const char** which);
diff --git a/elevenrender_amd/csrc/er_stream.hip b/elevenrender_amd/csrc/er_stream.hip
--- a/elevenrender_amd/csrc/er_stream.hip
+++ b/elevenrender_amd/csrc/er_stream.hip
@@ -998,7 +998,9 @@
     unsigned t5 = 0, t6 = 0, t7 = 0;
     if (COUNT) { t5 = st_wave_sum(c_nodes); t6 = st_wave_sum(c_tris); t7 = st_wave_sum(c_texels); }
     if (lane == 0) {
-        atomicMax((unsigned long long*)(status + ER_SC_END + 2 * (blockIdx.x & 7u)), (unsigned long long)wall_clock64());
+        const unsigned long long t_end = (unsigned long long)wall_clock64();
+        atomicMax((unsigned long long*)(status + ER_SC_END + 2 * (blockIdx.x & 7u)), t_end);
+        atomicMax((unsigned long long*)(status + ER_SC_WG_END + 2 * blockIdx.x), t_end);
         if (t0) atomicAdd(&S.counters->paths, (unsigned long long)t0);
         if (t1) atomicAdd(&S.counters->bounce_samples, (unsigned long long)t1);
         if (t2) atomicAdd(&S.counters->rays, (unsigned long long)t2);
diff --git a/elevenrender_amd/csrc/er_stream_host.cpp b/elevenrender_amd/csrc/er_stream_host.cpp
--- a/elevenrender_amd/csrc/er_stream_host.cpp
+++ b/elevenrender_amd/csrc/er_stream_host.cpp
@@ -47,6 +47,62 @@
             out[(size_t)b + (size_t)k * blocks] = seq[x][sidx];
         }
     return maxk;
+}
+
+uint32_t er_stream_level_by_cost(const std::vector<uint32_t>& deal, uint32_t tiles_x, uint32_t blocks, const uint32_t* cost, size_t cost_n, uint32_t cap, std::vector<uint32_t>& out) {
+    (void)tiles_x;
+    const uint32_t NONE = 0xFFFFFFFFu;
+    const uint32_t rows = blocks ? (uint32_t)(deal.size() / blocks) : 0u;
+    auto keep = [&]() { out = deal; return rows; };
+    if (!blocks || !rows || !cap) return keep();
+    const uint32_t X = blocks % 8u == 0u ? 8u : 1u, per = blocks / X;
+    auto c_of = [&](uint32_t t) -> uint64_t { return (cost && t < cost_n) ? cost[t] : 0u; };
+    std::vector<std::vector<uint32_t>> seq(X);
+    std::vector<uint64_t> sum(X, 0);
+    uint64_t total = 0;
+    for (uint32_t k = 0; k < rows; k++)
+        for (uint32_t j = 0; j < per; j++)
+            for (uint32_t x = 0; x < X; x++) {
+                const uint32_t t = deal[(size_t)(j * X + x) + (size_t)k * blocks];
+                if (t == NONE) continue;
+                seq[x].push_back(t); sum[x] += c_of(t); total += c_of(t);
+            }
+    if (total == 0) return keep();
+    for (uint32_t x = 0; x < X; x++) if (seq[x].size() > (size_t)per * cap) return keep();
+    for (;;) {
+        uint32_t hi = 0, lo = 0;
+        for (uint32_t x = 1; x < X; x++) {
+            if (sum[x] > sum[hi]) hi = x;
+            if (sum[x] < sum[lo]) lo = x;
+        }
+        if (hi == lo || seq[hi].empty() || seq[lo].size() >= (size_t)per * cap) break;
+        const uint32_t t = seq[hi].back();
+        const uint64_t c = c_of(t);
+        if (c == 0 || sum[hi] - sum[lo] <= 2u * c) break;
+        seq[hi].pop_back(); seq[lo].push_back(t);
+        sum[hi] -= c; sum[lo] += c;
+    }
+    std::vector<std::vector<uint32_t>> mine(blocks);
+    std::vector<uint64_t> load(per);
+    uint32_t most = 0;
+    for (uint32_t x = 0; x < X; x++) {
+        std::vector<uint32_t>& q = seq[x];
+        std::sort(q.begin(), q.end(), [&](uint32_t a, uint32_t b) { const uint64_t ca = c_of(a), cb = c_of(b); return ca != cb ? ca > cb : a < b; });
+        std::fill(load.begin(), load.end(), 0);
+        for (uint32_t t : q) {
+            uint32_t best = per;
+            for (uint32_t j = 0; j < per; j++)
+                if (mine[(size_t)j * X + x].size() < cap && (best == per || load[j] < load[best])) best = j;
+            if (best == per) return keep();
+            mine[(size_t)best * X + x].push_back(t);
+            load[best] += c_of(t);
+        }
+    }
+    for (auto& m : mine) { std::sort(m.begin(), m.end()); most = std::max<uint32_t>(most, (uint32_t)m.size()); }
+    out.assign((size_t)blocks * most, NONE);
+    for (uint32_t b = 0; b < blocks; b++)
+        for (size_t k = 0; k < mine[b].size(); k++) out[(size_t)b + k * blocks] = mine[b][k];
+    return most;
 }
 
 bool stream_xcd_aware(size_t owned_tiles, uint32_t blocks) {
@@ -87,8 +143,10 @@
 
 static hipError_t stream_drop_pending_deal(ErScene* s) {
     s->st.deal_pending = false;
+    s->st.counting = false;
     s->dev.tile_cost = s->ad_dev.tile_cost = nullptr;
     s->st.deal_large.clear(); s->st.deal_large.shrink_to_fit();
+    s->st.deal_base.clear(); s->st.deal_base.shrink_to_fit();
     return hipMemcpyAsync(s->d_dev.p, &s->dev, sizeof(DevScene), hipMemcpyHostToDevice, s->stream);
 }
 
@@ -101,16 +159,22 @@
     st.readings = 0;
     const size_t slots = (size_t)st.blocks * ER_STREAM_SLOTS, npx = (size_t)s->x_res * s->y_res;
     if ((rc = upload(s->d_wf4, nullptr, slots * er_stream_record_bytes(light_query) / sizeof(float4), s->stream)) != ER_OK) return rc;
-    if ((rc = upload(s->d_wf1, nullptr, ER_STREAM_CTL_LEAD + ER_SC_WORDS, s->stream)) != ER_OK) return rc;
+    const size_t ctl_words = ER_STREAM_CTL_LEAD + er_stream_ctl_words(st.blocks);
+    if ((rc = upload(s->d_wf1, nullptr, ctl_words, s->stream)) != ER_OK) return rc;
     if ((rc = upload(s->d_spill, nullptr, er_stream_spill_entries(st.blocks), s->stream)) != ER_OK) return rc;
     st.ctl = s->d_wf1.p;
-    HIP_TRY(hipMemsetAsync(st.ctl, 0, (ER_STREAM_CTL_LEAD + ER_SC_WORDS) * sizeof(uint32_t), s->stream));
+    HIP_TRY(hipMemsetAsync(st.ctl, 0, ctl_words * sizeof(uint32_t), s->stream));
     st.spec[0] = st.spec[1] = st.spec[2] = 0;
+    st.launch_start = st.launch_end = 0; st.wg_end.clear();
     const bool xcd_aware = stream_xcd_aware(owned.size(), st.blocks);
     const uint32_t tiles_x = s->tiles_x();
     uint32_t most = deal.most;
     st.deal_off = 0; st.deal_n = (uint32_t)deal.tiles.size();
     st.deal_alt_off = 0; st.deal_alt_n = 0;
+    st.deal_base_off = 0; st.deal_lvl_off = 0; st.deal_lvl_cap = 0; st.deal_levelled = false;
+    st.counting = false;
+    st.deal_base.clear(); st.cost_host.clear();
+    st.deal_host = deal.tiles;
     st.xcd_spread = -1.0;
     const char* adapt_knob = getenv("ER_STREAM_ADAPT");
     st.deal_pending = false;
@@ -128,12 +192,11 @@
             const size_t n_tiles = (size_t)tiles_x * s->tiles_y();
             if ((rc = upload(st.d_tile_cost, nullptr, n_tiles, s->stream)) != ER_OK) return rc;
             HIP_TRY(hipMemsetAsync(st.d_tile_cost.p, 0, n_tiles * sizeof(uint32_t), s->stream));
-            st.deal_pending = true;
+            st.deal_pending = st.counting = true;
         }
     }
     if ((rc = upload(st.d_px_draws, nullptr, npx, s->stream)) != ER_OK) return rc;
     HIP_TRY(hipMemsetAsync(st.d_px_draws.p, 0, npx * sizeof(uint32_t), s->stream));
-    if ((rc = upload(st.d_deal, deal.tiles.data(), deal.tiles.size(), s->stream)) != ER_OK) return rc;
     if (s->x_res > 65535u || s->y_res > 65535u)
         return fail(ER_ERR_INVALID_ARG, "er_render_begin: ER_FLAG_STREAM carries a pixel as x | y << 16: frames up to 65535 x 65535; use ER_FLAG_WAVEFRONT (the automatic choice does)");
     st.ring_cap = 64u;
@@ -142,13 +205,16 @@
         return fail(ER_ERR_INVALID_ARG, "er_render_begin: ER_FLAG_STREAM serves at most " + std::to_string((size_t)ER_STREAM_MAX_RING * st.blocks) +
                                             " owned pixels per rank; use ER_FLAG_WAVEFRONT (the automatic choice does)");
     if ((rc = upload(st.d_ticket, nullptr, (size_t)st.blocks * (size_t)st.ring_cap * 2, s->stream)) != ER_OK) return rc;
+    if (st.counting) { st.deal_lvl_off = (uint32_t)deal.tiles.size(); st.deal_lvl_cap = st.blocks * (st.ring_cap / 64u); }
+    if ((rc = upload(st.d_deal, nullptr, deal.tiles.size() + st.deal_lvl_cap, s->stream)) != ER_OK) return rc;
+    if (!deal.tiles.empty()) HIP_TRY(hipMemcpyAsync(st.d_deal.p, deal.tiles.data(), deal.tiles.size() * sizeof(uint32_t), hipMemcpyHostToDevice, s->stream));
     return ER_OK;
 }
 
 int stream_redeal(ErScene* s) {
     StreamHost& st = s->st;
     const bool large = st.large_deal_in_use();
-    if (st.deal_pending) HIP_TRY(stream_drop_pending_deal(s));
+    if (st.deal_pending || st.counting) HIP_TRY(stream_drop_pending_deal(s));
     const uint32_t count = (uint32_t)s->ad_active.size(), tiles_x = s->tiles_x();
     std::vector<uint32_t> deal;
     uint32_t most = er_stream_deal_tiles(s->ad_active.data(), count, tiles_x, st.blocks, stream_xcd_aware(count, st.blocks), deal, large ? ER_STREAM_SUPER_TILE_LARGE : 0u);
@@ -158,6 +224,8 @@
     if ((rc = upload(st.d_deal, deal.data(), deal.size(), s->stream)) != ER_OK) return rc;
     st.deal_off = 0; st.deal_n = (uint32_t)deal.size();
     st.deal_alt_off = 0; st.deal_alt_n = 0;
+    st.deal_base_off = 0; st.deal_lvl_off = 0; st.deal_lvl_cap = 0; st.deal_levelled = false;
+    st.deal_host = deal;
     stream_set_form(s, count);
     HIP_TRY(hipStreamSynchronize(s->stream));
     return ER_OK;
@@ -165,7 +233,7 @@
 
 static int stream_launch(ErScene* s, uint32_t k) {
     StreamHost& st = s->st;
-    HIP_TRY(hipMemsetAsync(st.status() + ER_SC_ITERS, 0, (ER_SC_WORDS - ER_SC_ITERS) * sizeof(uint32_t), s->stream));
+    HIP_TRY(hipMemsetAsync(st.status() + ER_SC_ITERS, 0, (er_stream_ctl_words(st.blocks) - ER_SC_ITERS) * sizeof(uint32_t), s->stream));
     HIP_TRY(hipMemsetAsync(st.status() + ER_SC_START, 0xFF, 2 * sizeof(uint32_t), s->stream));
     if (k > 0) st.launches++;
     ErStreamLaunch L;
@@ -203,8 +271,8 @@
 int er_scene_stream_status(ErScene* s, const char* who) {
     StreamHost& st = s->st;
     if (!(s->params.flags & ER_FLAG_STREAM) || !st.ctl) return ER_OK;
-    uint32_t w[ER_SC_WORDS] = {0};
-    HIP_TRY(hipMemcpy(w, st.status(), sizeof(w), hipMemcpyDeviceToHost));
+    std::vector<uint32_t> w(er_stream_ctl_words(st.blocks), 0u);
+    HIP_TRY(hipMemcpy(w.data(), st.status(), w.size() * sizeof(uint32_t), hipMemcpyDeviceToHost));
     if (st.spec_seen != st.launches) {
         st.spec_seen = st.launches;
         for (int k = 0; k < 3; k++) st.spec[k] += w[ER_SC_SPEC + k];
@@ -219,7 +287,45 @@
     for (uint32_t x = 0; x < 8; x++) { const unsigned long long e = u64(ER_SC_END + 2 * x); lo = std::min(lo, e); hi = std::max(hi, e); }
     st.xcd_spread = (t0 != ~0ull && lo > t0 && hi - t0 >= 200000ull) ? (double)(hi - lo) / (double)(hi - t0) : -1.0;
     st.launch_ms = (t0 != ~0ull && hi > t0) ? (double)(hi - t0) * 1e-5 : 0.0;
+    st.launch_start = (t0 != ~0ull && hi > t0) ? t0 : 0u; st.launch_end = st.launch_start ? hi : 0u;
+    st.wg_end.assign(st.blocks, 0u);
+    for (uint32_t b = 0; b < st.blocks; b++) st.wg_end[b] = u64(ER_SC_WG_END + 2 * b);
     return ER_OK;
+}
+
+void stream_balance(const ErScene* s, std::vector<uint32_t>& wg_tiles, std::vector<uint64_t>& wg_cost, std::vector<uint64_t>& wg_ticks) {
+    const StreamHost& st = s->st;
+    wg_tiles.assign(st.blocks, 0u); wg_cost.assign(st.blocks, 0u); wg_ticks.assign(st.blocks, 0u);
+    for (size_t i = 0; i < st.deal_host.size() && st.blocks; i++) {
+        const uint32_t t = st.deal_host[i];
+        if (t == 0xFFFFFFFFu) continue;
+        wg_tiles[i % st.blocks]++;
+        if (t < st.cost_host.size()) wg_cost[i % st.blocks] += st.cost_host[t];
+    }
+    for (uint32_t b = 0; b < st.blocks && b < st.wg_end.size(); b++)
+        if (st.launch_start && st.wg_end[b] > st.launch_start) wg_ticks[b] = st.wg_end[b] - st.launch_start;
+}
+
+static void stream_print_balance(const ErScene* s) {
+    const StreamHost& st = s->st;
+    std::vector<uint32_t> tiles; std::vector<uint64_t> cost, ticks;
+    stream_balance(s, tiles, cost, ticks);
+    double t_sum = 0, t_max = 0, t_min = 0, c_sum = 0, c_max = 0, c_min = 0;
+    uint32_t n = 0, n_max = 0, n_min = 0;
+    for (uint32_t b = 0; b < st.blocks; b++) {
+        if (!tiles[b] || !ticks[b]) continue;
+        const double t = (double)ticks[b], c = (double)cost[b];
+        if (!n) { t_max = t_min = t; c_max = c_min = c; n_max = n_min = tiles[b]; }
+        t_sum += t; t_max = std::max(t_max, t); t_min = std::min(t_min, t);
+        c_sum += c; c_max = std::max(c_max, c); c_min = std::min(c_min, c);
+        n_max = std::max(n_max, tiles[b]); n_min = std::min(n_min, tiles[b]);
+        n++;
+    }
+    if (!n || t_sum <= 0) return;
+    const double t_mean = t_sum / n, c_mean = c_sum / n;
+    fprintf(stderr, "[er_stream] workgroups of a launch of %.3f ms: finished max/mean %.4f min/mean %.4f, idle tail S %.4f", t_max * 1e-5, t_max / t_mean, t_min / t_mean, (t_max - t_mean) / t_max);
+    if (c_mean > 0) fprintf(stderr, "; counted cost max/mean %.4f min/mean %.4f", c_max / c_mean, c_min / c_mean);
+    fprintf(stderr, " (%s deal, %u ... %u tiles; measured times: printed, nothing is decided on them)\n", st.deal_levelled ? "cost-levelled" : "count", n_min, n_max);
 }
 
 void stream_adapt(ErScene* s) {
@@ -229,9 +335,17 @@
     if (st.adapted == st.launches) return;
     st.adapted = st.launches;
     if (verbose && !st.form.adapt) fprintf(stderr, "[er_stream] tracer lanes %.3f full at %u + %u waves (fixed split)\n", st.busy, st.form.tracers, st.form.waves - st.form.tracers);
+    const bool counted = st.deal_pending || st.counting;
+    bool have_cost = false;
+    if (counted) {
+        std::vector<uint32_t> cost(st.d_tile_cost.n);
+        have_cost = hipMemcpy(cost.data(), st.d_tile_cost.p, cost.size() * sizeof(uint32_t), hipMemcpyDeviceToHost) == hipSuccess;
+        if (have_cost) st.cost_host.swap(cost);
+    }
+    if (verbose) stream_print_balance(s);
     if (st.deal_pending) {
-        std::vector<uint32_t> cost(st.d_tile_cost.n);
-        if (hipMemcpy(cost.data(), st.d_tile_cost.p, cost.size() * sizeof(uint32_t), hipMemcpyDeviceToHost) == hipSuccess) {
+        const std::vector<uint32_t>& cost = st.cost_host;
+        if (have_cost) {
             double x[8] = {0, 0, 0, 0, 0, 0, 0, 0};
             const std::vector<uint32_t>& L = st.deal_large;
             for (size_t i = 0; i < L.size(); i++)
@@ -245,9 +359,29 @@
             st.cost_spread = spread;
             if (verbose) fprintf(stderr, "[er_stream] counted work of the XCDs' shares on super-tiles of %u: %.4f of the mean apart (limit %.4f) -> %s\n", (unsigned)ER_STREAM_SUPER_TILE_LARGE, spread,
                                  limit, take ? "large regions" : "the default deal stays");
-            if (take) { st.deal_off = st.deal_alt_off; st.deal_n = st.deal_alt_n; }
-        }
-        (void)stream_drop_pending_deal(s);
+            if (take) { st.deal_off = st.deal_base_off = st.deal_alt_off; st.deal_n = st.deal_alt_n; st.deal_host = st.deal_large; }
+        }
+        st.deal_pending = false;
+        st.deal_base = st.deal_host;
+        st.deal_large.clear(); st.deal_large.shrink_to_fit();
+    }
+    if (counted) {
+        const char* lv = getenv("ER_STREAM_COST_LEVEL");
+        const bool level = !(lv && atoi(lv) == 0) && have_cost && st.deal_lvl_cap != 0u && !st.deal_base.empty();
+        if (level) {
+            std::vector<uint32_t> lvl;
+            er_stream_level_by_cost(st.deal_base, s->tiles_x(), st.blocks, st.cost_host.data(), st.cost_host.size(), st.ring_cap / 64u, lvl);
+            if (lvl == st.deal_base) {
+                st.deal_off = st.deal_base_off; st.deal_n = (uint32_t)st.deal_base.size(); st.deal_levelled = false;
+                st.deal_host = st.deal_base;
+            } else if (lvl.size() <= st.deal_lvl_cap &&
+                       hipMemcpyAsync(st.d_deal.p + st.deal_lvl_off, lvl.data(), lvl.size() * sizeof(uint32_t), hipMemcpyHostToDevice, s->stream) == hipSuccess) {
+                (void)hipStreamSynchronize(s->stream);
+                st.deal_off = st.deal_lvl_off; st.deal_n = (uint32_t)lvl.size(); st.deal_levelled = true;
+                st.deal_host.swap(lvl);
+            }
+        }
+        if (!level || !st.probe_launch) (void)stream_drop_pending_deal(s);
         (void)hipStreamSynchronize(s->stream);
     }
     if (verbose && st.xcd_spread >= 0.0)
diff --git a/elevenrender_amd/csrc/er_stream_host.h b/elevenrender_amd/csrc/er_stream_host.h
--- a/elevenrender_amd/csrc/er_stream_host.h
+++ b/elevenrender_amd/csrc/er_stream_host.h
@@ -35,6 +35,8 @@
     uint32_t* status() const { return ctl + ER_STREAM_CTL_LEAD; }
     double busy = 0.0;
     double launch_ms = 0.0;
+    uint64_t launch_start = 0, launch_end = 0;
+    std::vector<uint64_t> wg_end;
     double xcd_spread = 0.0;
     double cost_spread = -1.0;
     uint64_t spec[3] = {0, 0, 0};
@@ -44,12 +46,19 @@
     erh::DevBuf<uint32_t> d_deal, d_ticket;
     uint32_t deal_off = 0, deal_n = 0;
     uint32_t deal_alt_off = 0, deal_alt_n = 0;
+    uint32_t deal_base_off = 0;
+    uint32_t deal_lvl_off = 0, deal_lvl_cap = 0;
+    bool deal_levelled = false;
+    bool counting = false;
+    std::vector<uint32_t> deal_base;
+    std::vector<uint32_t> deal_host;
+    std::vector<uint32_t> cost_host;
     bool deal_pending = false;
     erh::DevBuf<uint32_t> d_tile_cost;
     std::vector<uint32_t> deal_large;
     erh::DevBuf<uint32_t> d_px_draws;
 
-    bool large_deal_in_use() const { return deal_alt_n != 0u && deal_off == deal_alt_off; }
+    bool large_deal_in_use() const { return deal_alt_n != 0u && deal_base_off == deal_alt_off; }
     void release() {
         d_deal.release(); d_ticket.release(); d_tile_cost.release(); d_px_draws.release();
         ctl = nullptr;
@@ -61,3 +70,4 @@
 int stream_enqueue(ErScene* s, uint32_t n);
 void stream_adapt(ErScene* s);
 void stream_fill_info(const ErScene* s, ErStreamInfo* out);
+void stream_balance(const ErScene* s, std::vector<uint32_t>& wg_tiles, std::vector<uint64_t>& wg_cost, std::vector<uint64_t>& wg_ticks);
diff --git a/elevenrender_amd/render.py b/elevenrender_amd/render.py
--- a/elevenrender_amd/render.py
+++ b/elevenrender_amd/render.py
@@ -149,6 +149,18 @@
         abi.check(self.lib.er_debug_stream_info(self.handle, C.byref(si)))
         return {n: getattr(si, n) for n, _ in abi.ErStreamInfo._fields_}
 
+    def stream_balance(self):
+        info = abi.ErStreamBalance()
+        abi.check(self.lib.er_debug_stream_balance(self.handle, C.byref(info), None, None, None, 0, None, 0, None, 0))
+        b = info.blocks
+        ticks, tiles, cost = np.zeros(b, np.uint64), np.zeros(b, np.uint32), np.zeros(b, np.uint64)
+        deal, tile_cost = np.zeros(b * info.most, np.uint32), np.zeros(info.cost_tiles, np.uint32)
+        u32, u64 = (lambda a: a.ctypes.data_as(C.POINTER(C.c_uint32))), (lambda a: a.ctypes.data_as(C.POINTER(C.c_uint64)))
+        abi.check(self.lib.er_debug_stream_balance(self.handle, C.byref(info), u64(ticks), u32(tiles), u64(cost), b, u32(deal), deal.size, u32(tile_cost), tile_cost.size))
+        d = {n: int(getattr(info, n)) for n, _ in abi.ErStreamBalance._fields_}
+        d.update(wg_ticks=ticks, wg_tiles=tiles, wg_cost=cost, deal=deal.reshape(info.most, b) if b else deal, tile_cost=tile_cost)
+        return d
+
     def accel_info(self):
         a = abi.ErAccelInfo()
         abi.check(self.lib.er_accel_info(self.handle, C.byref(a)))
diff --git a/include/eleven_hip_debug.h b/include/eleven_hip_debug.h
--- a/include/eleven_hip_debug.h
+++ b/include/eleven_hip_debug.h
@@ -93,6 +93,21 @@
 int er_debug_stream_deal(const uint32_t* owned, uint32_t count, uint32_t tiles_x, uint32_t blocks, int xcd_aware, uint32_t edge, uint32_t* out, uint32_t out_cap,
                          uint32_t* most);
 
+int er_debug_stream_level(const uint32_t* deal, uint32_t deal_n, uint32_t tiles_x, uint32_t blocks, const uint32_t* cost, uint32_t cost_n, uint32_t cap,
+                          uint32_t* out, uint32_t out_cap, uint32_t* most);
+
+typedef struct ErStreamBalance {
+    uint32_t blocks;
+    uint32_t most;
+    uint32_t levelled;
+    uint32_t counting;
+    uint32_t cost_tiles;
+    uint32_t cap;
+    uint64_t launch_ticks;
+} ErStreamBalance;
+int er_debug_stream_balance(struct ErScene* s, ErStreamBalance* info, uint64_t* wg_ticks, uint32_t* wg_tiles, uint64_t* wg_cost, uint32_t wg_cap,
+                            uint32_t* deal, uint32_t deal_cap, uint32_t* tile_cost, uint32_t cost_cap);
+
 typedef struct ErStreamForm {
     uint32_t waves, tracers;
     uint32_t adapt;
```

After: 2067 Msamples/s (median of 6 runs). +2.1%, better.
